# RolandFaure/Hairsplitter

Hardware: AMD Instinct MI355X
Metric: aligned read-bp/sec through call_variants+separate_reads (higher is better)
Workload: dtype u8

## Files before the change

hairsplitter_amd/api.py:

```python
from __future__ import annotations

import ctypes as C
import os
from typing import Dict, List, Optional, Sequence

import numpy as np

from .dist import mean_of_positive_f32, stage4_error_rate, window_size_counts, window_size_from_counts

_ROOT = os.path.dirname(os.path.abspath(__file__))
LIB_PATH = os.path.join(_ROOT, "lib", "libhairsplitter_hip.so")
if os.environ.get("HS_LIB_AB"):
    LIB_PATH = os.environ["HS_LIB_AB"]

SYMBOLS = [
    "hs_cv_batch_set_ploidy", "hs_version", "hs_last_error", "hs_device_count", "hs_warmup", "hs_set_device", "hs_device_synchronize", "hs_malloc", "hs_free",
    "hs_memcpy_h2d", "hs_memcpy_d2h", "hs_memset", "hs_event_create", "hs_event_destroy", "hs_event_record",
    "hs_event_elapsed_ms", "hs_pileup", "hs_pileup_plan", "hs_free_host", "hs_tile_plan", "hs_column_stats_tiled", "hs_cv_column_pass_taps", "hs_cv_taps_destroy", "hs_cv_pileup_tap", "hs_cv_pileup_tap_destroy", "hs_sr_run_taps", "hs_sr_taps_destroy", "hs_exclusive_scan_i32", "hs_gaf_from_files", "hs_gaf_from_labels", "hs_gro_to_gaf_main", "hs_column_partition_test", "hs_column_partition_last_counts", "hs_loop_a_test", "hs_loop_a_result_destroy", "hs_partition_pair_distance", "hs_snp_planes", "hs_simdiff", "hs_read_graphs",
    "hs_edit_distance", "hs_cv_batch_create", "hs_cv_batch_destroy", "hs_cv_batch_aligned_bp", "hs_cv_run",
    "hs_cv_result_destroy", "hs_cv_select", "hs_cv_run_range", "hs_cv_selection_destroy", "hs_sr_run", "hs_sr_run_cv", "hs_sr_run_cv_range", "hs_pipeline_create", "hs_pipeline_select", "hs_pipeline_run", "hs_pipeline_destroy", "hs_pipeline_thread_devices", "hs_cv_batch_device", "hs_sr_result_destroy", "hs_sr_window_size", "hs_call_variants_main", "hs_call_variants_epilogue",
    "hs_pipeline_run_fused", "hs_realign_paf", "hs_pipeline_set_option", "hs_pipeline_groups", "hs_pipeline_group_range", "hs_pipeline_group_cv", "hs_pipeline_sparse_labels", "hs_separate_reads_main", "hs_main_process_exits", "hs_kernel_name", "hs_kernel_stats_reset", "hs_kernel_stats_get", "hs_kernel_stats_every", "hs_host_wait_stats", "hs_devices", "hs_cv_run_host", "hs_edlib_hw_align", "hs_edlib_align", "hs_edlib_align_bytes", "hs_alignment_to_cigar", "hs_reattach_ends", "hs_trim_polished", "hs_reattach_ends_bytes", "hs_trim_polished_bytes", "hs_free_strings", "hs_cut_gfa", "hs_gfa_to_fasta", "hs_cut_gfa_main", "hs_gfa2fa_main",
    "hs_polish_inputs", "hs_polish_inputs_from_files", "hs_polish_result_destroy", "hs_polish_inputs_main",
    "hs_moves_to_cigar", "hs_realign_intervals", "hs_realign_records_destroy", "hs_cv_batch_create_paf", "hs_cv_batch_create_sam",
    "hs_allele_table_destroy", "hs_alleles_text", "hs_alleles_lds_capacity", "hs_group_alleles_layout", "hs_group_alleles", "hs_haplotype_alleles", "hs_pipeline_alleles",
# ... 516 lines not shown
    _fields_ = [("n_snps", C.c_int64), ("n_cw_instances", C.c_int64), ("n_graph_rows_host", C.c_int64),
                ("t_device_ms", C.c_double), ("t_host_ms", C.c_double), ("t_kernel_cv_ms", C.c_float * 4), ("t_kernel_k4_ms", C.c_float),
                ("t_kernel_sr_ms", C.c_float * 4), ("t_kernel_graph_ms", C.c_float),
                ("n_columns_extracted", C.c_int64), ("n_columns_downloaded", C.c_int64), ("n_columns_downloaded_late", C.c_int64),
                ("n_cw_sweeps", C.c_int64), ("cw_bytes", C.c_int64), ("graph_nnz", C.c_int64), ("n_graph_rows", C.c_int64), ("simdiff_bytes", C.c_int64)]


class PipelineGroups:

    def __init__(self, contigs, n_groups):
        self.flat = contigs if isinstance(contigs, FlatBatch) else FlatBatch(contigs)
        self.batch = CvBatch(self.flat)
        self.handle = C.c_void_p()
        _check(load().hs_pipeline_create(self.batch.handle, C.c_int32(n_groups), C.byref(self.handle)))
        self.aligned_bp = self.flat.aligned_bp
        self.total_len = int(self.flat.contig_off[-1])
        self._owns_batch = True

    def keep_columns(self, on=True):
        _check(load().hs_pipeline_set_option(self.handle, C.c_int32(1), C.c_int64(1 if on else 0)))

    def sparse_labels(self, on=True):
        _check(load().hs_pipeline_set_option(self.handle, C.c_int32(2), C.c_int64(1 if on else 0)))
        self._sparse = bool(on)

    def alleles(self, on=True):
        _check(load().hs_pipeline_set_option(self.handle, C.c_int32(4), C.c_int64(1 if on else 0)))
        self._alleles = bool(on)

    def recruits(self, on=True, params=None):
        if params is not None:
            _check(load().hs_pipeline_set_recruit_params(self.handle, C.byref(_recruit_params(params))))
        _check(load().hs_pipeline_set_option(self.handle, C.c_int32(8), C.c_int64(1 if on else 0)))
        self._recruits = bool(on)

    def _attach_sparse(self, sr):
        if getattr(self, "_recruits", False):
            tb = load().hs_pipeline_recruits(self.handle)
            if not tb:
                raise HsError("hs_pipeline_recruits: no table")
            sr["recruits"] = _recruit_table_to_dict(tb)
        if getattr(self, "_alleles", False):
            tb = load().hs_pipeline_alleles(self.handle)
            if not tb:
                raise HsError("hs_pipeline_alleles: no table")
            sr["alleles"] = _allele_table_to_dict(tb)
        if not getattr(self, "_sparse", False):
            return sr
        off, ids, lab = C.POINTER(C.c_int64)(), C.POINTER(C.c_int32)(), C.POINTER(C.c_int32)()
        nw, nr = C.c_int64(0), C.c_int64(0)
        _check(load().hs_pipeline_sparse_labels(self.handle, C.byref(off), C.byref(ids), C.byref(lab), C.byref(nw), C.byref(nr)))
        W, R = int(nw.value), int(nr.value)
        if R == 0:
            sr["sparse"] = (np.ctypeslib.as_array(off, (W + 1,)), np.zeros(0, np.int32), np.zeros(0, np.int32))
            return sr
        sr["sparse"] = (np.ctypeslib.as_array(off, (W + 1,)), np.ctypeslib.as_array(ids, (R,)), np.ctypeslib.as_array(lab, (R,)))
        return sr

    def sibling(self, n_groups):
        o = object.__new__(PipelineGroups)
        o.flat, o.batch, o.aligned_bp, o.total_len = self.flat, self.batch, self.aligned_bp, self.total_len
        o.handle = C.c_void_p()
        o._owns_batch = False
        _check(load().hs_pipeline_create(self.batch.handle, C.c_int32(n_groups), C.byref(o.handle)))
        return o

    def run(self, automatic_snp_threshold=0.33, n_threads=0, error_rate_fn=None, rarest_strain_abundance=0.01, low_memory=False,
            amplicon=False, seed=12345, window_size=0):
        import time
        lib = load()
        Cn = self.flat.n_contigs
        md = np.zeros(max(Cn, 1), np.float32)
        st = PipelineStats()
        t_0 = time.perf_counter()
        _check(lib.hs_pipeline_select(self.handle, _hp(md, C.c_float), C.byref(st)))
        t_1 = time.perf_counter()
        md = md[:Cn]
        cv = {"mean_distance": md, "error_rate": mean_of_positive_f32(md)}
        e = error_rate_fn(cv) if error_rate_fn is not None else stage4_error_rate(cv["error_rate"])
        sres = C.POINTER(SrResult)()
        t_2 = time.perf_counter()
        _check(lib.hs_pipeline_run(self.handle, C.c_float(automatic_snp_threshold), C.c_float(e), C.c_float(rarest_strain_abundance),
                                   C.c_int32(1 if low_memory else 0), C.c_int32(1 if amplicon else 0), C.c_uint32(seed), C.c_int32(n_threads),
                                   C.c_int32(window_size), C.byref(sres), C.byref(st)))
        t_3 = time.perf_counter()
        cv.update({"n_snps": int(st.n_snps), "t_device_ms": float(st.t_device_ms), "t_host_ms": float(st.t_host_ms),
                   "t_kernel_ms": [float(x) for x in st.t_kernel_cv_ms], "t_kernel_k4_ms": float(st.t_kernel_k4_ms),
                   "n_columns_extracted": int(st.n_columns_extracted), "n_columns_downloaded": int(st.n_columns_downloaded),
                   "n_columns_downloaded_late": int(st.n_columns_downloaded_late)})
        sr = self._attach_sparse(_sr_result_to_dict(sres, Cn, take_ownership=True))
        sr["wall_ms"] = {"select": (t_1 - t_0) * 1e3, "between": (t_2 - t_1) * 1e3, "groups": (t_3 - t_2) * 1e3, "collect": (time.perf_counter() - t_3) * 1e3}
        return cv, sr

    def run_fused(self, automatic_snp_threshold=0.33, n_threads=0, rarest_strain_abundance=0.01, low_memory=False, amplicon=False, seed=12345,
                  window_size=0):
        import time
        lib = load()
        Cn = self.flat.n_contigs
        md = np.zeros(max(Cn, 1), np.float32)
        st = PipelineStats()
        er = C.c_float(0)
        sres = C.POINTER(SrResult)()
        t_0 = time.perf_counter()
        _check(lib.hs_pipeline_run_fused(self.handle, C.c_float(automatic_snp_threshold), C.c_float(rarest_strain_abundance), C.c_int32(1 if low_memory else 0),
                                         C.c_int32(1 if amplicon else 0), C.c_uint32(seed), C.c_int32(n_threads), C.c_int32(window_size), _hp(md, C.c_float),
                                         C.byref(er), C.byref(sres), C.byref(st)))
        t_1 = time.perf_counter()
        cv = {"mean_distance": md[:Cn], "error_rate": float(er.value), "error_rate_is_final": True, "n_snps": int(st.n_snps), "t_device_ms": float(st.t_device_ms),
              "t_host_ms": float(st.t_host_ms), "t_kernel_ms": [float(x) for x in st.t_kernel_cv_ms], "t_kernel_k4_ms": float(st.t_kernel_k4_ms),
              "n_columns_extracted": int(st.n_columns_extracted), "n_columns_downloaded": int(st.n_columns_downloaded),
              "n_columns_downloaded_late": int(st.n_columns_downloaded_late)}
        sr = self._attach_sparse(_sr_result_to_dict(sres, Cn, take_ownership=True))
        sr["wall_ms"] = {"select": 0.0, "between": 0.0, "groups": (t_1 - t_0) * 1e3, "collect": (time.perf_counter() - t_1) * 1e3}
        return cv, sr

    def window_size(self, amplicon=False):
        f = self.flat
        if amplicon:
            return int(np.diff(f.contig_off).max()) if f.n_contigs else 0
        return window_size_from_counts(*window_size_counts(f.rec_refspan + 2))

    def close(self):
        if self.handle:
            load().hs_pipeline_destroy(self.handle)
            self.handle = None
        if getattr(self, "_owns_batch", True):
            self.batch.close()


class _SrResultOwner:

    def __init__(self, res):
        self.res = res

    def __del__(self):
        try:
            load().hs_sr_result_destroy(self.res)
        except Exception:
            pass


class _SrTaps(C.Structure):
    _fields_ = [("n_windows", C.c_int32), ("win_contig", C.POINTER(C.c_int32)), ("win_start", C.POINTER(C.c_int32)), ("win_row0", C.POINTER(C.c_int64)),
                ("mask_ids", C.POINTER(C.c_int32)), ("run_begin", C.POINTER(C.c_int64)), ("run_snp", C.POINTER(C.c_int32)), ("run_off", C.POINTER(C.c_int64)),
                ("run_labels", C.POINTER(C.c_int32)), ("third", C.POINTER(C.c_int32)),
                ("g_n_windows", C.c_int32), ("g_win_contig", C.POINTER(C.c_int32)), ("g_win_kind", C.POINTER(C.c_int32)), ("g_win_row0", C.POINTER(C.c_int64)),
                ("g_mask_ids", C.POINTER(C.c_int32)), ("g_nbr_off", C.POINTER(C.c_int64)), ("g_nbr", C.POINTER(C.c_int32)), ("g_n_contigs", C.c_int32),
                ("g_plane_n", C.POINTER(C.c_int32)), ("g_words", C.POINTER(C.c_int32)), ("g_plane_off", C.POINTER(C.c_int64)), ("g_alt", C.POINTER(C.c_uint64)),
                ("g_ref", C.POINTER(C.c_uint64)), ("g_n_reads", C.POINTER(C.c_int32)), ("g_out_off", C.POINTER(C.c_int64)), ("g_read_base", C.POINTER(C.c_int64)),
                ("g_pos_orig", C.POINTER(C.c_int32)), ("g_n_pos_orig", C.c_int64), ("g_n_plane_words", C.c_int64), ("g_n_pairs", C.c_int64),
                ("g_matrix", C.POINTER(C.c_int32)), ("g_rows_on_host", C.c_int64), ("g_rows_late", C.c_int64), ("g_row_waves", C.c_int32),
                ("all_lanes", C.c_int32), ("cap_tail", C.c_int32), ("runs_lanes", C.c_int64), ("runs_overflow", C.c_int64), ("runs_rows", C.c_int64),
                ("units_rows", C.c_int64), ("runs_wave", C.c_int64), ("runs_wave_scratch", C.c_int64), ("tail_narrow", C.c_int64), ("tail_lds", C.c_int64),
                ("tail_scratch", C.c_int64)]


SR_ROUTE_COUNTERS = ("all_lanes", "runs_lanes", "runs_overflow", "runs_rows", "units_rows", "runs_wave", "runs_wave_scratch", "tail_narrow", "tail_lds",
                     "tail_scratch", "cap_tail")


SR_TAP_SENTINEL = -2 ** 31


def _sr_run_taps_fn(lib):
    lib.hs_sr_run_taps.argtypes = [C.c_void_p, C.c_int32, C.c_int32, C.c_float, C.c_int32, C.c_uint32, C.c_int32, C.c_int32, C.POINTER(C.POINTER(SrResult)),
                                   C.POINTER(C.POINTER(_SrTaps))]
    lib.hs_sr_taps_destroy.argtypes = [C.POINTER(_SrTaps)]; lib.hs_sr_taps_destroy.restype = None
    return lib.hs_sr_run_taps


def _graph_taps_to_dict(t):
    a = lambda ptr, n, dt: np.ctypeslib.as_array(ptr, (max(n, 1),))[:n].astype(dt).copy()
    W, Cn = int(t.g_n_windows), int(t.g_n_contigs)
    row0 = a(t.g_win_row0, W + 1, np.int64)
    rows = int(row0[-1])
    noff = a(t.g_nbr_off, rows + 1, np.int64)
    return {"win_contig": a(t.g_win_contig, W, np.int32), "win_kind": a(t.g_win_kind, W, np.int32), "win_row0": row0, "mask_ids": a(t.g_mask_ids, rows, np.int32),
            "nbr_off": noff, "nbr": a(t.g_nbr, int(noff[-1]), np.int32),
            "plane_n": a(t.g_plane_n, Cn, np.int32), "words": a(t.g_words, Cn, np.int32), "plane_off": a(t.g_plane_off, Cn, np.int64),
            "alt": a(t.g_alt, int(t.g_n_plane_words), np.uint64), "ref": a(t.g_ref, int(t.g_n_plane_words), np.uint64),
            "n_reads": a(t.g_n_reads, Cn, np.int32), "out_off": a(t.g_out_off, Cn, np.int64), "read_base": a(t.g_read_base, Cn, np.int64),
            "pos_orig": a(t.g_pos_orig, int(t.g_n_pos_orig), np.int32), "matrix": a(t.g_matrix, 2 * int(t.g_n_pairs), np.int32).reshape(-1, 2),
            "rows_on_host": int(t.g_rows_on_host), "rows_late": int(t.g_rows_late), "row_waves": int(t.g_row_waves)}


def _sr_contig_array(contigs):
    Cn = len(contigs)
    arr = (SrContig * max(Cn, 1))()
    keep = []
    for c, ctg in enumerate(contigs):
        rs, re = _np(ctg["read_start"], np.int32), _np(ctg["read_end"], np.int32)
        sp, sr, sa = _np(ctg["snp_pos"], np.int32), _np(ctg["snp_ref"], np.uint8), _np(ctg["snp_alt"], np.uint8)
        co, ci, cc = _np(ctg["col_off"], np.int64), _np(ctg["col_idx"], np.int32), _np(ctg["col_code"], np.uint8)
        if len(ci) == 0:
            ci, cc = np.zeros(1, np.int32), np.zeros(1, np.uint8)
        keep += [rs, re, sp, sr, sa, co, ci, cc]
        a = arr[c]
        a.length = int(ctg["length"]); a.n_reads = len(rs); a.n_snps = len(sp)
        a.read_start = _hp(rs, C.c_int32); a.read_end = _hp(re, C.c_int32)
        a.snp_pos = _hp(sp, C.c_int32); a.snp_ref = _hp(sr, C.c_uint8); a.snp_alt = _hp(sa, C.c_uint8)
        a.col_off = _hp(co, C.c_int64); a.col_idx = _hp(ci, C.c_int32); a.col_code = _hp(cc, C.c_uint8)
        a.ploidy = 0
    return arr, keep


def separate_reads_graph_taps(contigs: Sequence[Dict], window_size: int, error_rate: float, low_memory: bool = False, seed: int = 12345,
                              n_threads: int = 0) -> Dict:
    require_gpu()
    lib = load()
    Cn = len(contigs)
    arr, keep = _sr_contig_array(contigs)
    res = C.POINTER(SrResult)()
    tp = C.POINTER(_SrTaps)()
    _check(_sr_run_taps_fn(lib)(C.cast(arr, C.c_void_p), C.c_int32(Cn), C.c_int32(int(window_size)), C.c_float(error_rate), C.c_int32(1 if low_memory else 0),
                                C.c_uint32(seed), C.c_int32(n_threads), C.c_int32(1), C.byref(res), C.byref(tp)))
    out = _graph_taps_to_dict(tp.contents)
    lib.hs_sr_taps_destroy(tp)
    return out


def _chain_taps_to_dict(t):
    a = lambda ptr, n, dt: np.ctypeslib.as_array(ptr, (max(n, 1),))[:n].astype(dt).copy()
    Wc = int(t.n_windows)
    row0 = a(t.win_row0, Wc + 1, np.int64); rb = a(t.run_begin, Wc + 1, np.int64)
    n_runs = int(rb[-1]); ro = a(t.run_off, n_runs + 1, np.int64)
    out = {"win_contig": a(t.win_contig, Wc, np.int32), "win_start": a(t.win_start, Wc, np.int32), "win_row0": row0, "mask_ids": a(t.mask_ids, int(row0[-1]), np.int32),
           "run_begin": rb, "run_snp": a(t.run_snp, n_runs, np.int32), "run_off": ro, "run_labels": a(t.run_labels, int(ro[-1]), np.int32),
           "third": a(t.third, int(row0[-1]), np.int32)}
    for k in SR_ROUTE_COUNTERS:
        out[k] = int(getattr(t, k))
    return out


def separate_reads_chain_taps(contigs: Sequence[Dict], window_size: int, error_rate: float, low_memory: bool = False, seed: int = 12345,
                              n_threads: int = 0) -> Dict:
    require_gpu()
    lib = load()
    Cn = len(contigs)
    arr, keep = _sr_contig_array(contigs)
    res = C.POINTER(SrResult)()
    tp = C.POINTER(_SrTaps)()
    _check(_sr_run_taps_fn(lib)(C.cast(arr, C.c_void_p), C.c_int32(Cn), C.c_int32(int(window_size)), C.c_float(error_rate), C.c_int32(1 if low_memory else 0),
                                C.c_uint32(seed), C.c_int32(n_threads), C.c_int32(0), C.byref(res), C.byref(tp)))
    out = _sr_result_to_dict(res, Cn)
    out["window_size"] = int(window_size)
    lib.hs_sr_result_destroy(res)
    out["taps"] = _chain_taps_to_dict(tp.contents)
    lib.hs_sr_taps_destroy(tp)
    return out


def _sr_result_to_dict(res, Cn, take_ownership=False):
    r = res.contents
    win_off = np.ctypeslib.as_array(r.win_off, (Cn + 1,)).copy()
    W = int(win_off[-1])
    label_off = np.ctypeslib.as_array(r.label_off, (W + 1,)).copy()
    NL = int(label_off[-1])
    return {
        "win_off": win_off,
        "win_start": np.ctypeslib.as_array(r.win_start, (max(W, 1),))[:W].copy(),
        "win_end": np.ctypeslib.as_array(r.win_end, (max(W, 1),))[:W].copy(),
        "label_off": label_off,
        "labels": (None if not r.labels else (_owned_view_i32(res, r.labels, NL) if take_ownership else np.ctypeslib.as_array(r.labels, (max(NL, 1),))[:NL].copy())),
        "_owner": (_SrResultOwner(res) if (take_ownership and not r.labels) else None),
        "t_device_ms": float(r.t_device_ms), "t_host_ms": float(r.t_host_ms), "n_cw_instances": int(r.n_cw_instances),
        "t_kernel_ms": [float(x) for x in r.t_kernel_ms], "t_kernel_graph_ms": float(r.t_kernel_graph_ms),
        "n_graph_rows_host": int(r.n_graph_rows_host), "n_windows_finished_on_host": int(r.n_windows_finished_on_host),
        "n_cw_sweeps": int(r.n_cw_sweeps), "cw_bytes": int(r.cw_bytes), "graph_nnz": int(r.graph_nnz), "n_graph_rows": int(r.n_graph_rows),
        "simdiff_bytes": int(r.simdiff_bytes),
    }


def _owned_view_i32(res, ptr, n):
    buf = (C.c_int32 * max(n, 1)).from_address(C.addressof(ptr.contents))
    buf._hs_owner = _SrResultOwner(res)
    return np.ctypeslib.as_array(buf)[:n]


def separate_reads(cv_out: Dict, flat: FlatBatch, error_rate: float, low_memory: bool = False, amplicon: bool = False,
                   seed: int = 12345, n_threads: int = 0, ploidy: Optional[Sequence[int]] = None,
                   rarest_strain_abundance: float = 0.0, window_size: Optional[int] = None, taps: bool = False, alleles: bool = False,
                   recruit=False) -> Dict:
    require_gpu()
    lib = load()
    Cn = flat.n_contigs
    arr = (SrContig * Cn)()
    keep = []
    per_contig = []
    ops = flat.cigar & 0xF
    lens = (flat.cigar >> 4).astype(np.int64)
    refc = np.where((ops == 0) | (ops == 2) | (ops == 7) | (ops == 8), lens, 0)
    csum = np.concatenate(([0], np.cumsum(refc)))
    span = csum[flat.rec_cig_off[1:]] - csum[flat.rec_cig_off[:-1]]
    for c in range(Cn):
        r0, r1 = int(flat.contig_rec_off[c]), int(flat.contig_rec_off[c + 1])
        rs = _np(flat.rec_pos[r0:r1], np.int32)
        re = _np(flat.rec_pos[r0:r1].astype(np.int64) + 1 + span[r0:r1], np.int32)
        s0, s1 = int(cv_out["snp_off"][c]), int(cv_out["snp_off"][c + 1])
        e0 = int(cv_out["col_off"][s0])
        snp_pos = _np(cv_out["snp_pos"][s0:s1], np.int32)
        snp_ref = _np(cv_out["snp_ref"][s0:s1], np.uint8)
        snp_alt = _np(cv_out["snp_alt"][s0:s1], np.uint8)
        col_off = _np(cv_out["col_off"][s0:s1 + 1] - e0, np.int64)
        e1 = e0 + int(col_off[-1])
        col_idx = _np(cv_out["col_idx"][e0:e1], np.int32)
        col_code = _np(cv_out["col_code"][e0:e1], np.uint8)
        if rarest_strain_abundance > 0 and s1 > s0:
            seg = np.repeat(np.arange(s1 - s0), np.diff(col_off))
            n_ref = np.bincount(seg, weights=(col_code == snp_ref[seg]), minlength=s1 - s0)
            n_alt = np.bincount(seg, weights=(col_code == snp_alt[seg]) & (col_code != snp_ref[seg]), minlength=s1 - s0)
            keep_snp = n_alt.astype(np.float32) >= np.float32(rarest_strain_abundance) * (n_ref + n_alt).astype(np.float32)
            if not keep_snp.all():
                km = keep_snp[seg]
                lens = np.diff(col_off)[keep_snp]
                snp_pos, snp_ref, snp_alt = snp_pos[keep_snp], snp_ref[keep_snp], snp_alt[keep_snp]
                col_idx, col_code = _np(col_idx[km], np.int32), _np(col_code[km], np.uint8)
                col_off = _np(np.concatenate(([0], np.cumsum(lens))), np.int64)
                snp_pos, snp_ref, snp_alt = _np(snp_pos, np.int32), _np(snp_ref, np.uint8), _np(snp_alt, np.uint8)
                s1 = s0 + len(snp_pos)
        keep += [rs, re, snp_pos, snp_ref, snp_alt, col_off, col_idx, col_code]
        per_contig.append({"read_start": rs, "read_end": re, "snp_pos": snp_pos, "snp_ref": snp_ref, "snp_alt": snp_alt, "col_off": col_off, "col_idx": col_idx,
                           "col_code": col_code, "length": int(flat.contig_off[c + 1] - flat.contig_off[c])})
        a = arr[c]
        a.length = int(flat.contig_off[c + 1] - flat.contig_off[c])
        a.n_reads = r1 - r0
        a.read_start = _hp(rs, C.c_int32); a.read_end = _hp(re, C.c_int32)
        a.n_snps = s1 - s0
        a.snp_pos = _hp(snp_pos, C.c_int32); a.snp_ref = _hp(snp_ref, C.c_uint8); a.snp_alt = _hp(snp_alt, C.c_uint8)
        a.col_off = _hp(col_off, C.c_int64); a.col_idx = _hp(col_idx, C.c_int32); a.col_code = _hp(col_code, C.c_uint8)
        a.ploidy = int(ploidy[c]) if ploidy is not None else 0
    w = lib.hs_sr_window_size(arr, C.c_int32(Cn), C.c_int32(1 if amplicon else 0)) if window_size is None else int(window_size)
    if taps == "graphs":
        return {"window_size": int(w), "contigs": per_contig, "taps": separate_reads_graph_taps(per_contig, int(w), error_rate, low_memory, seed, n_threads)}
    res = C.POINTER(SrResult)()
    tp = C.POINTER(_SrTaps)()
    if taps:
        _check(_sr_run_taps_fn(lib)(C.cast(arr, C.c_void_p), C.c_int32(Cn), C.c_int32(w), C.c_float(error_rate), C.c_int32(1 if low_memory else 0),
                                    C.c_uint32(seed), C.c_int32(n_threads), C.c_int32(0), C.byref(res), C.byref(tp)))
    else:
        _check(lib.hs_sr_run(arr, C.c_int32(Cn), C.c_int32(w), C.c_float(error_rate), C.c_int32(1 if low_memory else 0),
                             C.c_uint32(seed), C.c_int32(n_threads), C.byref(res)))
    r = res.contents
    win_off = np.ctypeslib.as_array(r.win_off, (Cn + 1,)).copy()
    W = int(win_off[-1])
    label_off = np.ctypeslib.as_array(r.label_off, (W + 1,)).copy()
    NL = int(label_off[-1])
    out = {
        "window_size": int(w), "win_off": win_off,
        "win_start": np.ctypeslib.as_array(r.win_start, (max(W, 1),))[:W].copy(),
        "win_end": np.ctypeslib.as_array(r.win_end, (max(W, 1),))[:W].copy(),
        "label_off": label_off,
        "labels": np.ctypeslib.as_array(r.labels, (max(NL, 1),))[:NL].copy(),
        "t_device_ms": float(r.t_device_ms), "t_host_ms": float(r.t_host_ms), "n_cw_instances": int(r.n_cw_instances),
        "t_kernel_ms": [float(x) for x in r.t_kernel_ms], "t_kernel_graph_ms": float(r.t_kernel_graph_ms),
        "n_graph_rows_host": int(r.n_graph_rows_host), "n_windows_finished_on_host": int(r.n_windows_finished_on_host),
        "n_cw_sweeps": int(r.n_cw_sweeps), "cw_bytes": int(r.cw_bytes), "graph_nnz": int(r.graph_nnz), "n_graph_rows": int(r.n_graph_rows),
        "simdiff_bytes": int(r.simdiff_bytes),
    }
    if alleles:
        tb = C.POINTER(AlleleTable)()
        _check(lib.hs_haplotype_alleles(arr, C.c_int32(Cn), res, C.byref(tb)))
        out["alleles"] = _allele_table_to_dict(tb)
        lib.hs_allele_table_destroy(tb)
    if recruit:
        rt = C.POINTER(RecruitTable)()
        prm = _recruit_params(recruit if isinstance(recruit, dict) else None)
        _check(lib.hs_recruit_reads(arr, C.c_int32(Cn), res, C.byref(prm), None, C.byref(rt)))
        out["recruits"] = _recruit_table_to_dict(rt)
        lib.hs_recruit_table_destroy(rt)
    lib.hs_sr_result_destroy(res)
    if taps:
        out["taps"] = _chain_taps_to_dict(tp.contents)
        out["contigs"] = per_contig
        lib.hs_sr_taps_destroy(tp)
    return out


def alleles_lds_capacity() -> int:
    return int(load().hs_alleles_lds_capacity())


def _table_array(ptr, n, dtype) -> np.ndarray:
# ... 1169 lines not shown
```

hairsplitter_amd/csrc/hs_capi_multi.inc:

```
static std::vector<int> device_list() {
    std::vector<int> d;
    if (const char* e = std::getenv("HS_DEVICES")) {
        for (const char* p = e; *p;) { char* end = nullptr; const long v = std::strtol(p, &end, 10); if (end == p) break; d.push_back((int)v); p = *end == ',' ? end + 1 : end; }
    }
    int n = 0;
    if (hipGetDeviceCount(&n) != hipSuccess) n = 0;
    if (d.empty()) for (int i = 0; i < n; ++i) d.push_back(i);
    for (int& v : d) if (v < 0 || v >= n) v = 0;
    return d;
}
int hs_devices(int32_t* out, int32_t cap) {
    const std::vector<int> d = device_list();
    for (size_t i = 0; i < d.size() && (int32_t)i < cap; ++i) out[i] = d[i];
    return (int)d.size();
}
static std::vector<std::vector<int>> lpt_shards(const std::vector<double>& w, int parts) {
    std::vector<int> order(w.size());
    for (size_t i = 0; i < w.size(); ++i) order[i] = (int)i;
    std::sort(order.begin(), order.end(), [&](int a, int b) { return w[(size_t)a] != w[(size_t)b] ? w[(size_t)a] > w[(size_t)b] : a < b; });
    std::vector<double> load((size_t)parts, 0.0);
    std::vector<std::vector<int>> sh((size_t)parts);
    for (int i : order) {
        int best = 0;
        for (int k = 1; k < parts; ++k) if (load[(size_t)k] < load[(size_t)best]) best = k;
        sh[(size_t)best].push_back(i); load[(size_t)best] += w[(size_t)i];
    }
    for (auto& v : sh) std::sort(v.begin(), v.end());
    return sh;
}
static int run_on_devices(const std::vector<int>& devs, const std::function<int(int)>& f) {
    const int D = (int)devs.size();
    std::vector<int> rcs((size_t)D, 0);
    std::vector<std::string> errs((size_t)D);
    std::vector<std::thread> th;
    for (int k = 0; k < D; ++k)
        th.emplace_back([&, k] {
            if (hipSetDevice(devs[(size_t)k]) != hipSuccess) { rcs[(size_t)k] = HS_EHIP; errs[(size_t)k] = "hipSetDevice failed"; return; }
            set_wait_policy();
            rcs[(size_t)k] = f(k);
            if (rcs[(size_t)k]) errs[(size_t)k] = hs_last_error();
        });
    for (auto& t : th) t.join();
    for (int k = 0; k < D; ++k) if (rcs[(size_t)k]) { set_error(errs[(size_t)k]); return rcs[(size_t)k]; }
    return HS_OK;
}

void hs_sr_taps_destroy(hs_sr_taps* t) {
    if (!t) return;
    std::free(t->win_contig); std::free(t->win_start); std::free(t->win_row0); std::free(t->mask_ids); std::free(t->run_begin); std::free(t->run_snp); std::free(t->run_off);
    std::free(t->run_labels); std::free(t->third);
    std::free(t->g_win_contig); std::free(t->g_win_kind); std::free(t->g_win_row0); std::free(t->g_mask_ids); std::free(t->g_nbr_off); std::free(t->g_nbr);
    std::free(t->g_plane_n); std::free(t->g_words); std::free(t->g_plane_off); std::free(t->g_alt); std::free(t->g_ref); std::free(t->g_n_reads); std::free(t->g_out_off);
    std::free(t->g_read_base); std::free(t->g_pos_orig); std::free(t->g_matrix);
    std::free(t);
}
int hs_sr_run_taps(const hs_sr_contig* contigs, int32_t n_contigs, int32_t window_size, float error_rate, int32_t low_memory, uint32_t seed,
                   int32_t n_threads, int32_t mode, hs_sr_result** out, hs_sr_taps** taps) {
    if (int rc = require_device()) return rc;
    if (!out || !taps || n_contigs < 0 || (mode != HS_SR_TAPS_CHAIN && mode != HS_SR_TAPS_GRAPHS)) { set_error("hs_sr_run_taps: bad arguments"); return HS_EINVAL; }
    hs::SrTaps tp;
    tp.graphs = mode == HS_SR_TAPS_GRAPHS;
    {
        HipSrOps ops;
        if (int rc = hs::sr_run(ops, contigs, n_contigs, window_size, error_rate, low_memory, seed, n_threads, out, nullptr, nullptr, &tp)) return rc;
    }
    const size_t Wc = tp.win_contig.size();
    for (size_t k = 0; k < Wc; ++k) {
        const int64_t r0 = tp.win_row0[k], m = tp.win_row0[k + 1] - r0;
        for (int64_t i = tp.run_begin[k]; i < tp.run_begin[k + 1]; ++i)
            for (int64_t j = 0; j < m; ++j) { int32_t& l = tp.run_labels[(size_t)(tp.run_off[(size_t)i] + j)]; if (l >= 0 && l < m) l = tp.mask_ids[(size_t)(r0 + l)]; }
    }
    auto dup_vec = [](const auto& v) { using T = typename std::decay<decltype(v)>::type::value_type; T* p = (T*)std::malloc(std::max<size_t>(1, v.size()) * sizeof(T)); if (p && !v.empty()) std::memcpy(p, v.data(), v.size() * sizeof(T)); return p; };
    hs_sr_taps* t = (hs_sr_taps*)std::calloc(1, sizeof(hs_sr_taps));
    t->n_windows = (int32_t)Wc;
    t->win_contig = dup_vec(tp.win_contig); t->win_start = dup_vec(tp.win_start); t->win_row0 = dup_vec(tp.win_row0); t->mask_ids = dup_vec(tp.mask_ids);
    t->run_begin = dup_vec(tp.run_begin); t->run_snp = dup_vec(tp.run_snp); t->run_off = dup_vec(tp.run_off); t->run_labels = dup_vec(tp.run_labels); t->third = dup_vec(tp.third);
    {
        const hs::SrChainRoutes& rt = tp.routes;
        t->all_lanes = rt.all_lanes; t->cap_tail = rt.cap_tail; t->runs_lanes = rt.runs_lanes; t->runs_overflow = rt.runs_overflow; t->runs_rows = rt.runs_rows;
        t->units_rows = rt.units_rows; t->runs_wave = rt.runs_wave; t->runs_wave_scratch = rt.runs_wave_scratch; t->tail_narrow = rt.tail_narrow;
        t->tail_lds = rt.tail_lds; t->tail_scratch = rt.tail_scratch;
    }
    if (tp.graphs) {
        const hs::SrGraphTaps& f = tp.front;
        t->g_n_windows = (int32_t)f.win_contig.size();
        t->g_win_contig = dup_vec(f.win_contig); t->g_win_kind = dup_vec(f.win_kind); t->g_win_row0 = dup_vec(f.win_row0); t->g_mask_ids = dup_vec(f.mask_ids);
        t->g_nbr_off = dup_vec(f.nbr_off); t->g_nbr = dup_vec(f.nbr);
        t->g_n_contigs = (int32_t)f.plane_n.size();
        t->g_plane_n = dup_vec(f.plane_n); t->g_words = dup_vec(f.words); t->g_plane_off = dup_vec(f.plane_off); t->g_alt = dup_vec(f.alt); t->g_ref = dup_vec(f.ref);
        t->g_n_reads = dup_vec(f.n_reads); t->g_out_off = dup_vec(f.out_off); t->g_read_base = dup_vec(f.read_base); t->g_pos_orig = dup_vec(f.pos_orig);
        t->g_n_pos_orig = (int64_t)f.pos_orig.size(); t->g_n_plane_words = (int64_t)f.alt.size(); t->g_n_pairs = (int64_t)f.matrix.size() / 2;
        t->g_matrix = dup_vec(f.matrix);
        t->g_rows_on_host = f.rows_on_host; t->g_rows_late = f.rows_late; t->g_row_waves = f.row_waves;
    }
    *taps = t;
    return HS_OK;
}

int hs_sr_run(const hs_sr_contig* contigs, int32_t n_contigs, int32_t window_size, float error_rate, int32_t low_memory,
              uint32_t seed, int32_t n_threads, hs_sr_result** out) {
    if (int rc = require_device()) return rc;
    if (!out || n_contigs < 0) { set_error("hs_sr_run: bad arguments"); return HS_EINVAL; }
    const std::vector<int> devs = device_list();
    if (devs.size() <= 1 || n_contigs < 2) {
        HipSrOps ops;
        return hs::sr_run(ops, contigs, n_contigs, window_size, error_rate, low_memory, seed, n_threads, out);
    }
    std::vector<double> w((size_t)n_contigs);
    for (int c = 0; c < n_contigs; ++c) w[(size_t)c] = 16.0 * contigs[c].n_reads * (double)contigs[c].n_reads + (double)contigs[c].n_snps * contigs[c].n_reads + 1.0;
    const int D = (int)std::min<size_t>(devs.size(), (size_t)n_contigs);
    const std::vector<std::vector<int>> shards = lpt_shards(w, D);
    std::vector<hs_sr_result*> parts((size_t)D, nullptr);
    const int per = n_threads > 0 ? std::max(1, n_threads / D) : 0;
    const int rc = run_on_devices(std::vector<int>(devs.begin(), devs.begin() + D), [&](int k) {
        std::vector<hs_sr_contig> sub;
        for (int c : shards[(size_t)k]) sub.push_back(contigs[c]);
        HipSrOps ops;
        return hs::sr_run(ops, sub.data(), (int32_t)sub.size(), window_size, error_rate, low_memory, seed, per, &parts[(size_t)k]);
    });
    if (rc) { for (hs_sr_result* r : parts) if (r) hs::free_sr_result(r); return rc; }
    std::vector<std::pair<int, int>> where((size_t)n_contigs);
    for (int k = 0; k < D; ++k) for (size_t i = 0; i < shards[(size_t)k].size(); ++i) where[(size_t)shards[(size_t)k][i]] = std::make_pair(k, (int)i);
    hs_sr_result* R = (hs_sr_result*)std::calloc(1, sizeof(hs_sr_result));
    int64_t W = 0, NL = 0;
    for (hs_sr_result* r : parts) { W += r->win_off[r->n_contigs]; NL += r->label_off[r->win_off[r->n_contigs]]; }
    R->n_contigs = n_contigs;
    R->win_off = (int64_t*)std::malloc(((size_t)n_contigs + 1) * sizeof(int64_t));
    R->win_start = (int32_t*)std::malloc((size_t)std::max<int64_t>(1, W) * sizeof(int32_t));
    R->win_end = (int32_t*)std::malloc((size_t)std::max<int64_t>(1, W) * sizeof(int32_t));
    R->label_off = (int64_t*)std::malloc(((size_t)W + 1) * sizeof(int64_t));
    R->labels = hs::sr_labels_alloc((size_t)NL);
    R->win_off[0] = 0; R->label_off[0] = 0;
    std::vector<int64_t> lab0((size_t)n_contigs + 1, 0);
    for (int c = 0; c < n_contigs; ++c) {
        const hs_sr_result* r = parts[(size_t)where[(size_t)c].first];
        const int i = where[(size_t)c].second;
        R->win_off[c + 1] = R->win_off[c] + (r->win_off[i + 1] - r->win_off[i]);
        lab0[(size_t)c + 1] = lab0[(size_t)c] + (r->label_off[r->win_off[i + 1]] - r->label_off[r->win_off[i]]);
    }
    R->label_off[W] = NL;
    hs::hs_parallel_for(n_contigs, host_threads(), [&](int c) {
        const hs_sr_result* r = parts[(size_t)where[(size_t)c].first];
        const int i = where[(size_t)c].second;
        const int64_t q0 = r->win_off[i], nq = r->win_off[i + 1] - q0, w0 = R->win_off[c];
        if (nq == 0) return;
        std::memcpy(R->win_start + w0, r->win_start + q0, (size_t)nq * sizeof(int32_t));
        std::memcpy(R->win_end + w0, r->win_end + q0, (size_t)nq * sizeof(int32_t));
        const int64_t shift = lab0[(size_t)c] - r->label_off[q0];
        for (int64_t q = 0; q < nq; ++q) R->label_off[w0 + q] = r->label_off[q0 + q] + shift;
        std::memcpy(R->labels + lab0[(size_t)c], r->labels + r->label_off[q0], (size_t)(r->label_off[q0 + nq] - r->label_off[q0]) * sizeof(int32_t));
    });
    for (hs_sr_result* r : parts) {
        R->t_device_ms += r->t_device_ms; R->t_host_ms += r->t_host_ms; R->n_cw_instances += r->n_cw_instances;
        for (int k = 0; k < 4; ++k) R->t_kernel_ms[k] += r->t_kernel_ms[k];
        R->t_kernel_graph_ms += r->t_kernel_graph_ms; R->n_graph_rows_host += r->n_graph_rows_host; R->n_windows_finished_on_host += r->n_windows_finished_on_host;
        R->n_cw_sweeps += r->n_cw_sweeps; R->cw_bytes += r->cw_bytes; R->graph_nnz += r->graph_nnz; R->n_graph_rows += r->n_graph_rows; R->simdiff_bytes += r->simdiff_bytes;
        hs::free_sr_result(r);
    }
    *out = R;
    return HS_OK;
}

int hs_cv_run_host(const uint8_t* h_contig_seq, const int64_t* h_contig_off, int32_t n_contigs, const uint8_t* h_read_seq, const int64_t* h_read_off,
                   int32_t n_reads, const int32_t* h_rec_read, const int32_t* h_rec_pos, const uint8_t* h_rec_strand, const int64_t* h_rec_cig_off,
                   const uint32_t* h_cigar, const int32_t* h_contig_rec_off, float automatic_snp_threshold, int32_t n_threads, hs_cv_result** out) {
    if (int rc = require_device()) return rc;
    if (!out || n_contigs < 0) { set_error("hs_cv_run_host: bad arguments"); return HS_EINVAL; }
    const std::vector<int> devs = device_list();
    if (devs.size() <= 1 || n_contigs < 2) {
        hs_cv_batch* b = nullptr;
        if (int rc = hs_cv_batch_create(h_contig_seq, h_contig_off, n_contigs, h_read_seq, h_read_off, n_reads, h_rec_read, h_rec_pos, h_rec_strand,
                                        h_rec_cig_off, h_cigar, h_contig_rec_off, &b)) return rc;
        const int rc = hs_cv_run(b, automatic_snp_threshold, n_threads, out);
        hs_cv_batch_destroy(b);
        return rc;
    }
    std::vector<double> w((size_t)n_contigs, 1.0);
    for (int c = 0; c < n_contigs; ++c)
        for (int r = h_contig_rec_off[c]; r < h_contig_rec_off[c + 1]; ++r) w[(size_t)c] += (double)(h_read_off[h_rec_read[r] + 1] - h_read_off[h_rec_read[r]]);
    const int D = (int)std::min<size_t>(devs.size(), (size_t)n_contigs);
    const std::vector<std::vector<int>> shards = lpt_shards(w, D);
    std::vector<hs_cv_result*> parts((size_t)D, nullptr);
    const int per = n_threads > 0 ? std::max(1, n_threads / D) : 0;
    const int rc = run_on_devices(std::vector<int>(devs.begin(), devs.begin() + D), [&](int k) {
        const std::vector<int>& ids = shards[(size_t)k];
        std::vector<int64_t> c_off(1, 0), r_off(1, 0), cig_off(1, 0);
        std::vector<int32_t> rec_off(1, 0), rec_read, rec_pos;
        std::vector<uint8_t> rec_strand;
        std::vector<uint8_t, hs::NoInitAlloc<uint8_t>> c_seq, r_seq;
        std::vector<uint32_t, hs::NoInitAlloc<uint32_t>> cig;
        std::vector<int32_t> new_id((size_t)n_reads, -1);
        int n_sub_reads = 0;
        int64_t c_total = 0, r_total = 0, cig_total = 0, rec_total = 0;
        for (int c : ids) {
            c_total += h_contig_off[c + 1] - h_contig_off[c];
            for (int r = h_contig_rec_off[c]; r < h_contig_rec_off[c + 1]; ++r) {
                rec_total++; cig_total += h_rec_cig_off[r + 1] - h_rec_cig_off[r];
                if (new_id[(size_t)h_rec_read[r]] < 0) { new_id[(size_t)h_rec_read[r]] = n_sub_reads++; r_total += h_read_off[h_rec_read[r] + 1] - h_read_off[h_rec_read[r]]; }
            }
        }
        c_seq.resize((size_t)c_total); r_seq.resize((size_t)r_total); cig.resize((size_t)cig_total);
        rec_read.reserve((size_t)rec_total); rec_pos.reserve((size_t)rec_total); rec_strand.reserve((size_t)rec_total);
        r_off.assign((size_t)n_sub_reads + 1, 0);
        std::fill(new_id.begin(), new_id.end(), -1);
        n_sub_reads = 0;
        int64_t cw = 0, rw = 0, gw = 0;
        for (int c : ids) {
            const int64_t L = h_contig_off[c + 1] - h_contig_off[c];
            std::memcpy(c_seq.data() + cw, h_contig_seq + h_contig_off[c], (size_t)L); cw += L; c_off.push_back(cw);
            for (int r = h_contig_rec_off[c]; r < h_contig_rec_off[c + 1]; ++r) {
                const int g = h_rec_read[r];
                if (new_id[(size_t)g] < 0) {
                    new_id[(size_t)g] = n_sub_reads;
                    const int64_t n = h_read_off[g + 1] - h_read_off[g];
                    std::memcpy(r_seq.data() + rw, h_read_seq + h_read_off[g], (size_t)n); rw += n;
                    r_off[(size_t)++n_sub_reads] = rw;
                }
                rec_read.push_back(new_id[(size_t)g]); rec_pos.push_back(h_rec_pos[r]); rec_strand.push_back(h_rec_strand[r]);
                const int64_t n = h_rec_cig_off[r + 1] - h_rec_cig_off[r];
                std::memcpy(cig.data() + gw, h_cigar + h_rec_cig_off[r], (size_t)n * sizeof(uint32_t)); gw += n; cig_off.push_back(gw);
            }
            rec_off.push_back((int32_t)rec_read.size());
        }
        hs_cv_batch* b = nullptr;
        if (int rc2 = hs_cv_batch_create(c_seq.data(), c_off.data(), (int32_t)ids.size(), r_seq.data(), r_off.data(), n_sub_reads, rec_read.data(), rec_pos.data(),
                                         rec_strand.data(), cig_off.data(), cig.data(), rec_off.data(), &b)) return rc2;
        const int rc2 = hs_cv_run(b, automatic_snp_threshold, per, &parts[(size_t)k]);
        hs_cv_batch_destroy(b);
        return rc2;
    });
    if (rc) { for (hs_cv_result* r : parts) if (r) hs::free_cv_result(r); return rc; }
    std::vector<std::pair<int, int>> where((size_t)n_contigs);
    for (int k = 0; k < D; ++k) for (size_t i = 0; i < shards[(size_t)k].size(); ++i) where[(size_t)shards[(size_t)k][i]] = std::make_pair(k, (int)i);
    hs_cv_result* R = (hs_cv_result*)std::calloc(1, sizeof(hs_cv_result));
// ... 55 lines not shown
```

hairsplitter_amd/csrc/hs_driver.h:

```cpp
#pragma once
#include <cstdint>
#include <functional>
#include <vector>
#include "hs_host.h"
#include "hs_host_sr.h"

namespace hs {

struct CvMeta {
    int32_t n_contigs = 0, n_rec = 0;
    std::vector<int64_t> contig_off;
    std::vector<int32_t> contig_rec_off;
    std::vector<int64_t> pile_off;
    std::vector<int32_t> rec_pos;
    std::vector<int64_t> rec_refspan;
    int64_t total_len = 0;
    std::vector<int32_t> ploidy;
    std::vector<int32_t> rank_of, orig_of;
};

struct CvPartitionTest {
    std::vector<int32_t> contig_n_reads;
    std::vector<int32_t> part_off;
    std::vector<int64_t> part_state_off;
    std::vector<int8_t> part_state;
};

struct CvCandidates {
    int64_t n_columns = 0, n_entries = 0;
    int64_t n_tie = 0, n_tie_big = 0;
    std::vector<int32_t> contig_n_cand;
    std::vector<float> contig_mean_distance;
    int64_t n_cand = 0;
    const hs_colrec* rec = nullptr;
    const int32_t* col = nullptr;
    const int64_t* off = nullptr;
    const int32_t* idx = nullptr;
    const uint8_t* code = nullptr;
    const CandBits* bits = nullptr;
    const uint64_t* words = nullptr;
    std::vector<uint8_t> contig_on_device;
};
struct CvSnpSet {
    std::vector<int32_t> contig_n_snp;
    int64_t n_snp = 0, n_entries = 0;
    const hs_colrec* rec = nullptr;
    const int64_t* off = nullptr;
    const int32_t* idx = nullptr;
    const uint8_t* code = nullptr;
};

struct CvLoopAResult {
    std::vector<uint8_t> on_device;
    std::vector<int32_t> failed;
    std::vector<int64_t> part_base;
    const CvPartRecord* rec = nullptr;
    const uint64_t* bits = nullptr;
    const int32_t* cnt = nullptr;
};

struct CvDeviceOps {
    virtual ~CvDeviceOps() {}
    virtual int pileup(std::vector<int32_t>& rec_stats, float k_ms[4]) = 0;
    virtual int extract_candidates(int c0, int c1, const std::vector<int32_t>& min_reads, float automatic_snp_threshold, CvCandidates& out,
                                   float k_ms[3], bool want_entries = true) = 0;
    virtual int fetch_candidates(CvCandidates& out) { (void)out; return -1; }
    virtual int finish_columns(const CvPartitionTest& t, bool want_entries, CvSnpSet& out, float* k_ms) = 0;
    virtual int late_entries(CvSnpSet& out) { (void)out; return 0; }
    virtual bool has_partition_pairs() const { return false; }
    virtual int partition_pairs(const std::vector<int8_t>& state, const std::vector<int32_t>& more, const std::vector<int32_t>& less, const std::vector<int64_t>& part_off,
                                const std::vector<int32_t>& part_n, const std::vector<int32_t>& pair_a, const std::vector<int32_t>& pair_b, const std::vector<float>& sigma3,
                                std::vector<int32_t>& out) { (void)state; (void)more; (void)less; (void)part_off; (void)part_n; (void)pair_a; (void)pair_b; (void)sigma3; (void)out; return -1; }
    virtual int collect_partitions(CvLoopAResult& out) { out = CvLoopAResult(); return 0; }
};

struct CvSelection {
    std::vector<int32_t> rec_stats;
    float k_ms[4] = {0, 0, 0, 0};
    double t_device_ms = 0, t_host_ms = 0;
};
int cv_pileup(CvDeviceOps& dev, const CvMeta& meta, CvSelection& sel);
int cv_run_range(CvDeviceOps& dev, const CvMeta& meta, const std::vector<int32_t>& rec_stats, int c0, int c1, float automatic_snp_threshold, int n_threads,
                 hs_cv_result** out, bool resident = false, const std::function<void(const float*)>* on_mean_distance = nullptr);
int cv_run(CvDeviceOps& dev, const CvMeta& meta, float automatic_snp_threshold, int n_threads, hs_cv_result** out);
hs_cv_result* cv_concat_results(hs_cv_result* a, hs_cv_result* b);
int cv_attach_entries(CvDeviceOps& dev, hs_cv_result* r, int n_threads, bool borrow = false);

struct SrWindowSet {
    std::vector<int32_t> win_contig;
    std::vector<int64_t> win_row0;
    std::vector<int32_t> mask_ids;
    int32_t n_dev_windows = 0;
    int32_t n_matrix_windows = 0;
    std::vector<int32_t> ctg_reads;
    std::vector<int64_t> host_off;
    std::vector<int32_t> host_nbr;
    std::vector<uint8_t> win_final_empty;
    std::vector<int32_t> rank;
    std::vector<int32_t> pos_rank;
    std::vector<int64_t> ctg_rank_off;
    float error_rate = 0;
    int64_t rows() const { return win_row0.empty() ? 0 : win_row0.back(); }
};

template <class T> struct ArrayView {
    const T* p = nullptr;
    size_t n = 0;
    std::vector<T> own;
    void view(const T* ptr, size_t count) { own.clear(); p = ptr; n = count; }
    T* alloc(size_t count) { own.resize(count); p = own.data(); n = count; return own.data(); }
    const T* data() const { return p; }
    size_t size() const { return n; }
    const T& operator[](size_t i) const { return p[i]; }
};

struct CwChain {
    ArrayView<int64_t> col_off;
    ArrayView<int32_t> col_idx;
    ArrayView<uint8_t> col_code;
    std::vector<int32_t> win;
    std::vector<int64_t> chain_row0;
    std::vector<int64_t> win_seed_begin;
    std::vector<int64_t> seed_col;
    bool finish_on_device = false;
    std::vector<int32_t> col_pos;
    std::vector<int64_t> win_snp_first, win_snp_last;
    std::vector<int32_t> win_pos_lo, win_pos_hi;
};

struct CwWave {
    std::vector<int32_t> inst_win;
    std::vector<int64_t> inst_label_off;
    std::vector<int32_t> labels;
};

struct SimdiffJob {
    const CwChain* cols = nullptr;
    std::vector<uint8_t> snp_ref, snp_alt;
    std::vector<int32_t> snp_contig;
    std::vector<int64_t> contig_snp_base;
    std::vector<int64_t> plane_off, out_off;
    std::vector<int32_t> n_reads, words;
    std::vector<int32_t> plane_n;
    int64_t plane_total = 0, out_total = 0;
    std::vector<int32_t> pos_orig;
    std::vector<int64_t> read_base;
};

struct SrChainStats {
    int64_t n_instances = 0;
    int64_t sweeps = 0;
    int64_t bytes = 0;
    int64_t graph_nnz = 0;
};

struct SrGraphTaps;
struct SrChainRoutes {
    int32_t all_lanes = 0;
    int64_t runs_lanes = 0;
    int64_t runs_overflow = 0;
    int64_t runs_rows = 0;
    int64_t units_rows = 0;
    int64_t runs_wave = 0;
    int64_t runs_wave_scratch = 0;
    int64_t tail_narrow = 0;
    int64_t tail_lds = 0;
    int64_t tail_scratch = 0;
    int32_t cap_tail = 0;
};
struct SrDeviceOps {
    virtual ~SrDeviceOps() {}
    virtual int simdiff_columns(const SimdiffJob& job, float* k_ms) = 0;
    virtual int build_graphs(const SrWindowSet& ws, int64_t* rows_on_host, float* k_ms) = 0;
    virtual bool two_phase_graphs() const { return false; }
    virtual int build_graphs_begin(const SrWindowSet& ws, float* k_ms) { (void)ws; (void)k_ms; return -1; }
    virtual int build_graphs_end(const SrWindowSet& ws, int64_t* rows_on_host) { (void)ws; (void)rows_on_host; return -1; }
    virtual int fetch_graphs(std::vector<int64_t>& off, std::vector<int32_t>& nbr) = 0;
    virtual int cw_chain(const CwChain& chain, std::vector<int32_t>& labels, std::vector<int32_t>& final_labels,
                         std::vector<uint8_t>& final_ok, float k_ms[3], SrChainStats* stats) = 0;
    virtual int cw(CwWave& wave, float* k_ms) = 0;
    virtual void tap_chain(std::vector<int64_t>* run_off, std::vector<int32_t>* run_labels, SrChainRoutes* routes) { (void)run_off; (void)run_labels; (void)routes; }
    virtual void tap_front(SrGraphTaps* t) { (void)t; }
    virtual bool low_memory_graphs() const { return false; }
    virtual bool columns_resident() const { return false; }
    virtual void drop_resident_columns() {}
    virtual int window_masks(const std::vector<int64_t>& col_a, const std::vector<int64_t>& col_b, const std::vector<int64_t>& slot_off,
                             std::vector<int32_t>& ids, std::vector<int32_t>& win_m) { (void)col_a; (void)col_b; (void)slot_off; (void)ids; (void)win_m; return -1; }
    virtual int fetch_columns(std::vector<int32_t>& idx, std::vector<uint8_t>& code) { (void)idx; (void)code; return -1; }
};

void set_trace_origin();
double trace_ms();
int host_threads();

struct SrSparseLabels {
    std::vector<int64_t> off;
    std::vector<int32_t> ids, labels;
};
struct SrWorkspace { std::vector<SrContigState> st; };
struct SrGraphTaps {
    static constexpr int32_t kSentinel = INT32_MIN;
    std::vector<int32_t> win_contig, win_kind;
    std::vector<int64_t> win_row0;
    std::vector<int32_t> mask_ids;
    std::vector<int64_t> nbr_off;
    std::vector<int32_t> nbr;
    std::vector<int32_t> plane_n, words, n_reads;
    std::vector<int64_t> plane_off, out_off, read_base;
    std::vector<int32_t> pos_orig;
    std::vector<uint64_t> alt, ref;
    std::vector<int32_t> matrix;
    int64_t rows_on_host = 0, rows_late = 0;
    int32_t row_waves = 0;
};
struct SrTaps {
    std::vector<int32_t> win_contig, win_start;
    std::vector<int64_t> win_row0;
    std::vector<int32_t> mask_ids;
    std::vector<int64_t> run_begin;
    std::vector<int32_t> run_snp;
    std::vector<int64_t> run_off;
    std::vector<int32_t> run_labels, third;
    SrChainRoutes routes;
    bool graphs = false;
    SrGraphTaps front;
};
int sr_run(SrDeviceOps& dev, const hs_sr_contig* contigs, int32_t n_contigs, int32_t window_size, float error_rate,
           int32_t low_memory, uint32_t seed, int32_t n_threads, hs_sr_result** out, SrSparseLabels* sparse = nullptr, SrWorkspace* keep = nullptr, SrTaps* taps = nullptr);

inline bool snp_kept_by_abundance(int32_t n_ref, int32_t n_alt, float rarest_strain_abundance) {
    return (float)n_alt >= rarest_strain_abundance * (float)(n_ref + n_alt);
}
int sr_run_from_cv(SrDeviceOps& dev, const CvMeta& meta, int c0, int c1, const hs_cv_result* cv, float error_rate, float rarest_strain_abundance,
                   int32_t low_memory, int32_t amplicon, uint32_t seed, int32_t n_threads, int32_t window_size, hs_sr_result** out,
                   SrSparseLabels* sparse = nullptr, SrWorkspace* keep = nullptr);

int32_t* sr_labels_alloc(size_t n_labels);
void sr_labels_free(int32_t* labels);
void sr_expand_labels(const SrSparseLabels& sp, const int64_t* label_off, int64_t w0, int64_t w1, int32_t* dense);

struct ColFileContig {
    std::string contig_line, name;
    long length = 0;
    std::vector<std::string> read_lines;
    std::vector<int32_t> read_start, read_end;
    std::vector<int32_t> snp_pos;
    std::vector<uint8_t> snp_ref, snp_alt;
    std::vector<int64_t> col_off{0};
    std::vector<int32_t> col_idx;
    std::vector<uint8_t> col_code;
};
int parse_col(const std::string& path, float rarest_strain_abundance, std::vector<ColFileContig>& cs, int n_threads = 1);
int read_col_sidecar(const std::string& col_path, float rarest_strain_abundance, std::vector<ColFileContig>& cs, int n_threads = 1);

int write_cv_outputs(const CvFileInput& in, const hs_cv_result* res, const std::string& error_rate_out,
                     const std::string& col_path, const std::string& vcf_path, int n_threads = 1);
int write_gro(const std::vector<ColFileContig>& cs, const hs_sr_result* res, const std::string& path, int n_threads = 1);
int write_gro_companion(const std::string& col_path, const std::vector<ColFileContig>& cs, const hs_sr_result* res, float error_rate, float rsa, bool low_memory, bool amplicon,
                        uint32_t seed, int32_t window, int n_threads);
int take_gro_companion(const std::string& col_path, float error_rate, float rsa, bool low_memory, bool amplicon, uint32_t seed, const std::string& outfile, int n_threads);
void remove_gro_companion(const std::string& col_path);
bool mark_gro_companion_pending(const std::string& col_path, float error_rate, float rsa, bool low_memory, bool amplicon, uint32_t seed);

void free_cv_result(hs_cv_result* r);
void free_sr_result(hs_sr_result* r);

}
```

hairsplitter_amd/csrc/hs_kernels_cw.hip:

```cpp
#pragma once

namespace hsdev {

#define HS_FIN_KCAP 16
#define HS_FIN_GCAP 8
#define HS_FIN_LCAP 16
#define HS_FIN_MCAP (HS_FIN_KCAP + 2)
#define HS_TAIL_MAP_EXTRA 1024
#define HS_TAIL_BATCH 8
#define HS_CWR_CAP 255
#ifndef HS_CW_REG_LABELS
#define HS_CW_REG_LABELS 8
#endif

static __device__ __forceinline__ int local_index(const int32_t* __restrict__ ids, int m, int r) {
    int lo = 0, hi = m;
    while (lo < hi) { const int mid = (lo + hi) >> 1; if (ids[mid] < r) lo = mid + 1; else hi = mid; }
    return (lo < m && ids[lo] == r) ? lo : -1;
}

__global__ __launch_bounds__(256) void k_cw_visit_lists(
    const int64_t* __restrict__ off, const int32_t* __restrict__ nbr, const int64_t* __restrict__ win_row0, const int32_t* __restrict__ mask_ids,
    const int32_t* __restrict__ win_contig, const int64_t* __restrict__ ctg_rank_off, const int32_t* __restrict__ rank,
    int n_windows, int cap, int32_t* __restrict__ visit, int32_t* __restrict__ visit_n,
// ... 239 lines not shown
                const int nc = __builtin_amdgcn_readfirstlane((int)((inf >> 8) & 255u));
                const uint8_t* pg = s_prog + (inf >> 16) * 16 + l;
                unsigned best = 0u;
                const int old = (int)lab[i];
                if (nc == 1) {
                    const int n0 = pg[0];
                    const int lb = n0 != 255 ? (int)lab[n0] : -1;
                    int cnt = 1;
#define HS_ROT(K) { const int o = __builtin_amdgcn_update_dpp(-2, lb, 0x120 + (K), 0xf, 0xf, false); cnt += o == lb ? 1 : 0; }
                    HS_ROT(1) HS_ROT(2) HS_ROT(3) HS_ROT(4) HS_ROT(5) HS_ROT(6) HS_ROT(7) HS_ROT(8)
                    HS_ROT(9) HS_ROT(10) HS_ROT(11) HS_ROT(12) HS_ROT(13) HS_ROT(14) HS_ROT(15)
#undef HS_ROT
                    best = row_max_u32(lb >= 0 ? (((unsigned)cnt << 16) | (unsigned)(65535 - lb)) : 0u);
                } else if (nc <= 4) {
                    const int n0 = pg[0], n1 = pg[16], n2 = nc > 2 ? pg[32] : 255, n3 = nc > 3 ? pg[48] : 255;
                    int lb0 = n0 != 255 ? (int)lab[n0] : -1, lb1 = n1 != 255 ? (int)lab[n1] : -1;
                    int lb2 = n2 != 255 ? (int)lab[n2 & 255] : -1, lb3 = n3 != 255 ? (int)lab[n3 & 255] : -1;
                    const int sh = tid & 48;
                    bool left = true;
                    for (int round = 0; round < HS_CW_REG_LABELS; ++round) {
                        const int mine = lb0 >= 0 ? lb0 : (lb1 >= 0 ? lb1 : (lb2 >= 0 ? lb2 : lb3));
                        const unsigned key = row_max_u32((unsigned)(mine + 1));
                        if (__ballot(key != 0u) == 0ull) { left = false; break; }
                        const int X = (int)key - 1;
                        const unsigned long long b0 = __ballot(lb0 == X && X >= 0), b1 = __ballot(lb1 == X && X >= 0);
                        const unsigned long long b2 = __ballot(lb2 == X && X >= 0), b3 = __ballot(lb3 == X && X >= 0);
                        const int c = __popc((unsigned)(b0 >> sh) & 0xffffu) + __popc((unsigned)(b1 >> sh) & 0xffffu) + __popc((unsigned)(b2 >> sh) & 0xffffu)
                                    + __popc((unsigned)(b3 >> sh) & 0xffffu);
                        const unsigned k = X >= 0 ? (((unsigned)c << 16) | (unsigned)(65535 - X)) : 0u;
                        best = k > best ? k : best;
                        lb0 = lb0 == X ? -1 : lb0; lb1 = lb1 == X ? -1 : lb1; lb2 = lb2 == X ? -1 : lb2; lb3 = lb3 == X ? -1 : lb3;
                    }
                    if (left && __ballot((lb0 & lb1 & lb2 & lb3) >= 0 || lb0 >= 0 || lb1 >= 0 || lb2 >= 0 || lb3 >= 0) != 0ull) {
                        const int m0 = n0 != 255 ? (int)lab[n0] : -1, m1 = n1 != 255 ? (int)lab[n1] : -1, m2 = n2 != 255 ? (int)lab[n2 & 255] : -1, m3 = n3 != 255 ? (int)lab[n3 & 255] : -1;
                        best = 0u;
                        if (m0 >= 0) atomicAdd(&cnt[m0], 1);
                        if (m1 >= 0) atomicAdd(&cnt[m1], 1);
                        if (m2 >= 0) atomicAdd(&cnt[m2], 1);
                        if (m3 >= 0) atomicAdd(&cnt[m3], 1);
                        wave_lds_sync();
                        if (m0 >= 0) { const unsigned k = ((unsigned)cnt[m0] << 16) | (unsigned)(65535 - m0); best = k > best ? k : best; }
                        if (m1 >= 0) { const unsigned k = ((unsigned)cnt[m1] << 16) | (unsigned)(65535 - m1); best = k > best ? k : best; }
                        if (m2 >= 0) { const unsigned k = ((unsigned)cnt[m2] << 16) | (unsigned)(65535 - m2); best = k > best ? k : best; }
                        if (m3 >= 0) { const unsigned k = ((unsigned)cnt[m3] << 16) | (unsigned)(65535 - m3); best = k > best ? k : best; }
                        best = row_max_u32(best);
                        wave_lds_sync();
                        if (m0 >= 0) cnt[m0] = 0;
                        if (m1 >= 0) cnt[m1] = 0;
                        if (m2 >= 0) cnt[m2] = 0;
                        if (m3 >= 0) cnt[m3] = 0;
                    }
                } else {
                    for (int c = 0; c < nc; ++c) { const int nb = pg[c * 16]; if (nb != 255) atomicAdd(&cnt[lab[nb]], 1); }
                    wave_lds_sync();
                    for (int c = 0; c < nc; ++c) { const int nb = pg[c * 16]; if (nb != 255) { const int lb = lab[nb]; const unsigned k = ((unsigned)cnt[lb] << 16) | (unsigned)(65535 - lb); best = k > best ? k : best; } }
                    best = row_max_u32(best);
                    wave_lds_sync();
                    for (int c = 0; c < nc; ++c) { const int nb = pg[c * 16]; if (nb != 255) cnt[lab[nb]] = 0; }
                }
                const int best_lab = 65535 - (int)(best & 0xffffu);
                changes += old != best_lab ? 1 : 0;
                wave_lds_sync();
                if (l == 0 && active) lab[i] = (uint8_t)best_lab;
                wave_lds_sync();
                inf = inf_next;
            }
            if (active) { iters++; active = changes > 2 && iters < 15; }
        }
    } else {
        int changes = 3;
        while (live && changes > 2 && iters < 15) {
            changes = 0;
            for (int v = 0; v < n_visit; ++v) {
                const int i = vis[v];
                const int o0 = (int)(off_w[i] - base), o1 = (int)(off_w[i + 1] - base);
                unsigned best = 0u;
                for (int o = o0 + l; o < o1; o += 16) atomicAdd(&cnt[lab[anb[o]]], 1);
                wave_lds_sync();
                for (int o = o0 + l; o < o1; o += 16) { const int lb = lab[anb[o]]; const unsigned key = ((unsigned)cnt[lb] << 16) | (unsigned)(65535 - lb); best = key > best ? key : best; }
                best = row_max_u32(best);
                wave_lds_sync();
                for (int o = o0 + l; o < o1; o += 16) cnt[lab[anb[o]]] = 0;
                const int best_lab = 65535 - (int)(best & 0xffffu);
                if ((int)lab[i] != best_lab) changes++;
                wave_lds_sync();
                if (l == 0) lab[i] = (uint8_t)best_lab;
                wave_lds_sync();
            }
            iters++;
        }
    }
    if (live) {
        int32_t* __restrict__ out = slab + inst_slab_off[inst];
        for (int j = l; j < m; j += 16) out[j] = (int32_t)lab[j];
        if (l == 0 && stat) {
            atomicAdd(&stat[0], (unsigned long long)iters);
            atomicAdd(&stat[1], (unsigned long long)iters * (4ull * (unsigned long long)(off_w[m] - base) + 8ull * (unsigned long long)m));
            atomicAdd(&stat[4 + (iters > 15 ? 15 : iters)], 1ull);
        }
    }
}

__global__ __launch_bounds__(64) void k_cw_seeded_wave(
    const int64_t* __restrict__ off, const int32_t* __restrict__ nbr, const int64_t* __restrict__ win_row0,
    const int32_t* __restrict__ mask_ids, const int32_t* __restrict__ visit, const int32_t* __restrict__ visit_n,
    const int32_t* __restrict__ inst_list, int n_list, const int32_t* __restrict__ n_list_dev ,
    const int32_t* __restrict__ inst_win, const int64_t* __restrict__ inst_seed_col,
    const int64_t* __restrict__ inst_slab_off, const int64_t* __restrict__ col_off, const int32_t* __restrict__ col_idx,
    const uint8_t* __restrict__ col_code, int lds_cap, int32_t* __restrict__ gscratch, const int64_t* __restrict__ gscratch_off,
    int32_t* __restrict__ slab, unsigned long long* __restrict__ stat) {
    extern __shared__ int32_t cw_dyn[];
    __shared__ int32_t s_first[256];
    const int lane = lane_id();
    const int n_runs = n_list_dev ? *n_list_dev : n_list;
    for (int k = (int)blockIdx.x; k < n_runs; k += (int)gridDim.x) {
    wave_lds_sync();
    const int inst = inst_list[k];
    const int w = inst_win[inst];
    const int64_t r0 = win_row0[w];
    const int m = (int)(win_row0[w + 1] - r0);
    const int32_t* __restrict__ ids = mask_ids + r0;
    int32_t* lab = m <= lds_cap ? cw_dyn : gscratch + gscratch_off[k];
    int32_t* cnt = lab + (m <= lds_cap ? lds_cap : m);
    for (int j = lane; j < m; j += 64) { lab[j] = j; cnt[j] = 0; }
    for (int j = lane; j < 256; j += 64) s_first[j] = 0x7fffffff;
    wave_lds_sync();
    const int64_t s = inst_seed_col[inst];
    cw_seed_labels<64>(ids, m, col_off[s], col_off[s + 1], col_idx, col_code, s_first, lane);
    wave_lds_sync();
    for (int64_t e = col_off[s] + lane; e < col_off[s + 1]; e += 64) {
        const int j = local_index(ids, m, col_idx[e]);
        if (j >= 0) lab[j] = s_first[col_code[e]];
    }
    wave_lds_sync();
    const int iters = cw_local_wave(off + r0, nbr, visit + r0, visit_n[w], m, lab, cnt, lane);
    int32_t* __restrict__ out = slab + inst_slab_off[inst];
    for (int j = lane; j < m; j += 64) out[j] = lab[j];
    if (lane == 0 && stat) {
        atomicAdd(&stat[0], (unsigned long long)iters);
        atomicAdd(&stat[1], (unsigned long long)iters * (4ull * (unsigned long long)(off[r0 + m] - off[r0]) + 8ull * (unsigned long long)m));
        atomicAdd(&stat[4 + (iters > 15 ? 15 : iters)], 1ull);
    }
    }
}

#define HS_CWL_SLOTS 16

__global__ __launch_bounds__(256) void k_cw_seed_sets(
    const int64_t* __restrict__ win_row0, const int32_t* __restrict__ mask_ids, const int32_t* __restrict__ inst_list, int n_list,
    const int32_t* __restrict__ inst_win, const int64_t* __restrict__ inst_seed_col, const int64_t* __restrict__ col_off,
    const int32_t* __restrict__ col_idx, const uint8_t* __restrict__ col_code,
    unsigned long long* __restrict__ seed_sets , uint8_t* __restrict__ seed_names ,
    uint8_t* __restrict__ seed_slots , uint8_t* __restrict__ seed_n ,
    int32_t* __restrict__ ovf_list, int32_t* __restrict__ ovf_n) {
    __shared__ int32_t s_ids[4][64];
    __shared__ int32_t s_lab[4][64];
    __shared__ int32_t s_first[4][256];
    const int lane = (int)threadIdx.x & 63, wv = (int)threadIdx.x >> 6;
    const int q = (int)blockIdx.x * 4 + wv;
    if (q >= n_list) return;
    int32_t* ids = s_ids[wv]; int32_t* lab = s_lab[wv]; int32_t* first = s_first[wv];
    const int inst = inst_list[q];
    const int w = inst_win[inst];
    const int64_t seed = inst_seed_col[inst];
    const int64_t r0 = win_row0[w];
    const int m = (int)(win_row0[w + 1] - r0);
    const int64_t c0 = col_off[seed], c1 = col_off[seed + 1];
    const int64_t e0 = c0 + lane;
    const int R0 = e0 < c1 ? col_idx[e0] : -1;
    const int code0 = e0 < c1 ? (int)col_code[e0] : 0;
    ids[lane] = lane < m ? mask_ids[r0 + lane] : 0x7fffffff;
    lab[lane] = lane;
    for (int c = lane; c < 256; c += 64) first[c] = 0x7fffffff;
    wave_lds_sync();
    const int j0 = R0 >= 0 ? local_index(ids, m, R0) : -1;
    if (j0 >= 0) atomicMin(&first[code0], j0);
    for (int64_t e = e0 + 64; e < c1; e += 64) { const int j = local_index(ids, m, col_idx[e]); if (j >= 0) atomicMin(&first[col_code[e]], j); }
    wave_lds_sync();
    if (j0 >= 0) lab[j0] = first[code0];
    for (int64_t e = e0 + 64; e < c1; e += 64) { const int j = local_index(ids, m, col_idx[e]); if (j >= 0) lab[j] = first[col_code[e]]; }
    wave_lds_sync();
    const int L = lab[lane];
    const bool node = lane < m;
    const unsigned long long leaders = __ballot(node && L == lane);
    const int alive = __popcll(leaders);
    const int slot = __popcll(leaders & ((1ull << L) - 1ull));
    seed_slots[(int64_t)q * 64 + lane] = (uint8_t)(node ? slot : 0);
    if (alive > HS_CWL_SLOTS) {
        if (lane == 0) { seed_n[q] = 255; ovf_list[atomicAdd(ovf_n, 1)] = inst; }
        return;
    }
    unsigned long long mine = 0ull;
#pragma unroll
    for (int k = 0; k < HS_CWL_SLOTS; ++k) { const unsigned long long S = __ballot(node && slot == k); if (lane == k) mine = S; }
    if (lane < HS_CWL_SLOTS) seed_sets[(int64_t)q * HS_CWL_SLOTS + lane] = mine;
    if (node && L == lane) ids[slot] = lane;
    wave_lds_sync();
    if (lane < HS_CWL_SLOTS) seed_names[(int64_t)q * HS_CWL_SLOTS + lane] = (uint8_t)(lane < alive ? ids[lane] : 0);
    if (lane == 0) seed_n[q] = (uint8_t)alive;
}

template <int NS>
static __device__ __forceinline__ int cwl_sweeps(unsigned (&set_lo)[HS_CWL_SLOTS], unsigned (&set_hi)[HS_CWL_SLOTS], uint8_t* my_slot,
                                                 const unsigned long long* __restrict__ adj_w, const uint32_t* __restrict__ inf_w, int nv, bool ok) {
    int iters = 0;
    bool active = ok;
    while (__ballot(active) != 0ull) {
        int changes = 0;
        unsigned long long adj_n = (active && nv > 0) ? adj_w[0] : 0ull;
        uint32_t inf_n = (active && nv > 0) ? inf_w[0] : 0u;
        for (int v = 0;; ++v) {
            const bool on = active && v < nv;
            if (__ballot(on) == 0ull) break;
            const unsigned long long adj = adj_n;
            const int i = (int)(inf_n & 255u);
            if (active && v + 1 < nv) { adj_n = adj_w[v + 1]; inf_n = inf_w[v + 1]; }
            const int old = (int)my_slot[i];
            const unsigned lo = (unsigned)adj, hi = (unsigned)(adj >> 32);
            unsigned best = 0u;
#pragma unroll
            for (int s = 0; s < NS; ++s) {
                const unsigned c = (unsigned)__popc(lo & set_lo[s]) + (unsigned)__popc(hi & set_hi[s]);
                const unsigned key = (c << 8) | (unsigned)(255 - s);
                best = key > best ? key : best;
            }
            const int b = 255 - (int)(best & 255u);
            const bool chg = on && b != old;
            changes += chg ? 1 : 0;
            if (__ballot(chg) != 0ull) {
                const unsigned long long bit = chg ? 1ull << i : 0ull;
                const unsigned bl = (unsigned)bit, bh = (unsigned)(bit >> 32);
#pragma unroll
                for (int s = 0; s < NS; ++s) {
                    set_lo[s] = (set_lo[s] & ~bl) | (s == b ? bl : 0u);
                    set_hi[s] = (set_hi[s] & ~bh) | (s == b ? bh : 0u);
                }
                if (chg) my_slot[i] = (uint8_t)b;
            }
        }
        if (active) { iters++; active = changes > 2 && iters < 15; }
    }
    return iters;
}

__global__ __launch_bounds__(64) void k_cw_seeded_lanes(
    const int64_t* __restrict__ off, const int64_t* __restrict__ win_row0, const int32_t* __restrict__ visit_n,
    const uint32_t* __restrict__ prog_info, const unsigned long long* __restrict__ prog_adj,
    const int32_t* __restrict__ inst_list, int n_list, const int32_t* __restrict__ inst_win, const int64_t* __restrict__ inst_slab_off,
    const unsigned long long* __restrict__ seed_sets, const uint8_t* __restrict__ seed_names, const uint8_t* __restrict__ seed_slots ,
    const uint8_t* __restrict__ seed_n, int32_t* __restrict__ slab, unsigned long long* __restrict__ stat) {
    __shared__ uint32_t s_slot[64 * 17];
    __shared__ uint32_t s_name[64 * 4];
    __shared__ unsigned int s_hist[16];
    const int lane = (int)threadIdx.x;
    const int q0 = (int)blockIdx.x * 64, q = q0 + lane;
    const bool valid = q < n_list;
    const int inst = valid ? inst_list[q] : 0;
    const int na = valid ? (int)seed_n[q] : 255;
    const bool ok = valid && na != 255;
    const int w = ok ? inst_win[inst] : 0;
    const int64_t r0 = ok ? win_row0[w] : 0;
    const int m = ok ? (int)(win_row0[w + 1] - r0) : 0;
    const int nv = ok ? visit_n[w] : 0;
    const int64_t out0 = ok ? inst_slab_off[inst] : 0;
    unsigned set_lo[HS_CWL_SLOTS], set_hi[HS_CWL_SLOTS];
    {
        const ulonglong2* p = reinterpret_cast<const ulonglong2*>(seed_sets + (int64_t)(valid ? q : 0) * HS_CWL_SLOTS);
#pragma unroll
        for (int k = 0; k < HS_CWL_SLOTS / 2; ++k) {
            const ulonglong2 v = p[k];
            set_lo[2 * k] = ok ? (unsigned)v.x : 0u; set_hi[2 * k] = ok ? (unsigned)(v.x >> 32) : 0u;
            set_lo[2 * k + 1] = ok ? (unsigned)v.y : 0u; set_hi[2 * k + 1] = ok ? (unsigned)(v.y >> 32) : 0u;
        }
        const uint4 nm = reinterpret_cast<const uint4*>(seed_names)[valid ? q : 0];
        s_name[lane * 4 + 0] = nm.x; s_name[lane * 4 + 1] = nm.y; s_name[lane * 4 + 2] = nm.z; s_name[lane * 4 + 3] = nm.w;
        const uint32_t* src = reinterpret_cast<const uint32_t*>(seed_slots + (int64_t)q0 * 64);
#pragma unroll
        for (int k = 0; k < 16; ++k) { const int x = lane + 64 * k; s_slot[(x >> 4) * 17 + (x & 15)] = src[x]; }
        if (lane < 16) s_hist[lane] = 0u;
    }
    wave_lds_sync();
    int nmax = 0;
#pragma unroll
    for (int k = 1; k <= HS_CWL_SLOTS; ++k) if (__ballot(ok && na >= k) != 0ull) nmax = k;
    uint8_t* my_slot = reinterpret_cast<uint8_t*>(s_slot) + lane * 68;
    int iters;
    if (nmax <= 4) iters = cwl_sweeps<4>(set_lo, set_hi, my_slot, prog_adj + r0, prog_info + r0, nv, ok);
    else if (nmax <= 6) iters = cwl_sweeps<6>(set_lo, set_hi, my_slot, prog_adj + r0, prog_info + r0, nv, ok);
    else if (nmax <= 8) iters = cwl_sweeps<8>(set_lo, set_hi, my_slot, prog_adj + r0, prog_info + r0, nv, ok);
    else if (nmax <= 10) iters = cwl_sweeps<10>(set_lo, set_hi, my_slot, prog_adj + r0, prog_info + r0, nv, ok);
    else if (nmax <= 12) iters = cwl_sweeps<12>(set_lo, set_hi, my_slot, prog_adj + r0, prog_info + r0, nv, ok);
    else iters = cwl_sweeps<HS_CWL_SLOTS>(set_lo, set_hi, my_slot, prog_adj + r0, prog_info + r0, nv, ok);
    wave_lds_sync();
    const unsigned long long okm = __ballot(ok);
    const uint8_t* names = reinterpret_cast<const uint8_t*>(s_name);
    const uint8_t* slots = reinterpret_cast<const uint8_t*>(s_slot);
    const int out_lo = (int)(unsigned)out0, out_hi = (int)(out0 >> 32);
    for (int r = 0; r < 64; ++r) {
        if (!((okm >> r) & 1ull)) continue;
        const int m_r = __builtin_amdgcn_readlane(m, r);
        const int64_t o_r = (int64_t)(((unsigned long long)(unsigned)__builtin_amdgcn_readlane(out_hi, r) << 32) | (unsigned)__builtin_amdgcn_readlane(out_lo, r));
        if (lane < m_r) slab[o_r + lane] = (int32_t)names[r * 16 + slots[r * 68 + lane]];
    }
    if (stat) {
        unsigned long long sw = ok ? (unsigned long long)iters : 0ull;
        unsigned long long by = ok ? (unsigned long long)iters * (4ull * (unsigned long long)(off[r0 + m] - off[r0]) + 8ull * (unsigned long long)m) : 0ull;
        if (ok) atomicAdd(&s_hist[iters > 15 ? 15 : iters], 1u);
#pragma unroll
        for (int d = 32; d >= 1; d >>= 1) { sw += __shfl_xor(sw, d, 64); by += __shfl_xor(by, d, 64); }
        wave_lds_sync();
        if (lane == 0) { atomicAdd(&stat[0], sw); atomicAdd(&stat[1], by); }
        if (lane < 16 && s_hist[lane]) atomicAdd(&stat[4 + lane], (unsigned long long)s_hist[lane]);
    }
}

__global__ __launch_bounds__(64) void k_cw_local(
    const int64_t* __restrict__ off, const int32_t* __restrict__ nbr, const int64_t* __restrict__ win_row0,
    const int32_t* __restrict__ visit, const int32_t* __restrict__ visit_n, const uint8_t* __restrict__ win_final_empty,
    const int32_t* __restrict__ inst_win, const int64_t* __restrict__ inst_label_off, int n_inst, int lds_cap,
    int32_t* __restrict__ gscratch, const int64_t* __restrict__ gscratch_off, int32_t* __restrict__ labels_io) {
    extern __shared__ int32_t cw_dyn[];
    const int lane = lane_id();
    const int k = (int)blockIdx.x;
    if (k >= n_inst) return;
    const int w = inst_win[k];
    const int64_t r0 = win_row0[w];
    const int m = (int)(win_row0[w + 1] - r0);
    int32_t* lab = m <= lds_cap ? cw_dyn : gscratch + gscratch_off[k];
    int32_t* cnt = lab + (m <= lds_cap ? lds_cap : m);
    int32_t* __restrict__ io = labels_io + inst_label_off[k];
    for (int j = lane; j < m; j += 64) { lab[j] = io[j]; cnt[j] = 0; }
    wave_lds_sync();
    cw_local_wave(off + r0, nbr, visit + r0, win_final_empty[w] ? 0 : visit_n[w], m, lab, cnt, lane);
    for (int j = lane; j < m; j += 64) io[j] = lab[j];
}

static __device__ __forceinline__ unsigned long long sets_from_labels(int L, unsigned long long* s_sets, int lane) {
    s_sets[lane] = 0ull;
    wave_lds_sync();
    if (L >= 0) atomicOr(&s_sets[L], 1ull << lane);
    wave_lds_sync();
    const unsigned long long S = s_sets[lane];
    wave_lds_sync();
    return S;
}
static __device__ __forceinline__ int sets_renumber(unsigned long long& S, int& L, unsigned long long* s_sets, int* s_relabel, int lane) {
    const int f = S ? __builtin_ctzll(S) : 64;
    const unsigned long long F = wave_or_u64(S ? 1ull << f : 0ull);
    const int nl = S ? __popcll(F & ((1ull << f) - 1ull)) : -1;
    s_sets[lane] = 0ull; s_relabel[lane] = nl;
    wave_lds_sync();
    if (nl >= 0) s_sets[nl] = S;
    const int Ln = L >= 0 ? s_relabel[L] : -1;
    wave_lds_sync();
    S = s_sets[lane]; L = Ln;
    wave_lds_sync();
    return __popcll(F);
}
#define HS_CW_SPEC_LABELS 8
static __device__ int cw_run_sets(unsigned long long adjv, int nodev, unsigned long long adjn, int n_visit, unsigned long long& S, int& L, int lane) {
    int changes = 3, iters = 0;
    while (changes > 2 && iters < 15) {
        changes = 0;
        unsigned long long alive = __ballot(S != 0ull);
        if (__popcll(alive) > HS_CW_SPEC_LABELS) {
            for (int v = 0; v < n_visit; ++v) {
                const unsigned long long adj = readlane_u64(adjv, v);
                const int i = __builtin_amdgcn_readlane(nodev, v);
                const int c = __popcll(adj & S);
                const int best = wave_max_i32(c ? ((c << 6) | (63 - lane)) : 0);
                if (best) {
                    const int bl = 63 - (best & 63);
                    const int old = __builtin_amdgcn_readlane(L, i);
                    if (old != bl) {
                        changes++;
                        const unsigned long long bit = 1ull << i;
                        if (lane == old) S &= ~bit;
                        if (lane == bl) S |= bit;
                        if (lane == i) L = bl;
                    }
                }
            }
        } else {
            int p = 0;
            while (p < n_visit) {
                int best = 0;
                for (unsigned long long am = alive; am; am &= am - 1ull) {
                    const int l = __builtin_ctzll(am);
                    const int c = __popcll(adjn & readlane_u64(S, l));
                    const int key = c ? ((c << 6) | (63 - l)) : 0;
                    best = key > best ? key : best;
                }
                const int wants = 63 - (best & 63);
                const unsigned long long U = __ballot(best != 0 && wants != L);
                const unsigned long long Uv = __ballot(lane >= p && lane < n_visit && ((U >> nodev) & 1ull));
                if (!Uv) break;
                const int v0 = __builtin_ctzll(Uv);
                const int i = __builtin_amdgcn_readlane(nodev, v0);
                const int bl = __builtin_amdgcn_readlane(wants, i), old = __builtin_amdgcn_readlane(L, i);
                const unsigned long long bit = 1ull << i;
                if (lane == old) S &= ~bit;
                if (lane == bl) S |= bit;
                if (lane == i) L = bl;
                changes++;
                p = v0 + 1;
                alive = __ballot(S != 0ull);
            }
        }
        iters++;
    }
    return iters;
}

static __device__ void first_seen_ids_wave(const int32_t* first, int m, int32_t* pre, int32_t* out_id, int lane) {
    int carry = 0;
    for (int b0 = 0; b0 < m; b0 += 64) {
        const int j = b0 + lane;
        const bool f = j < m && first[j] == j;
        const unsigned long long b = __ballot(f);
        if (j < m) pre[j] = carry + __popcll(b & ((1ull << lane) - 1ull));
        carry += __popcll(b);
    }
    wave_lds_sync();
    for (int j = lane; j < m; j += 64) { const int f = first[j]; out_id[j] = f >= 0 ? pre[f] : -1; }
    wave_lds_sync();
}

__global__ __launch_bounds__(64) void k_window_tail(
    const int64_t* __restrict__ off, const int32_t* __restrict__ nbr, const int64_t* __restrict__ win_row0,
    const int32_t* __restrict__ mask_ids, const int32_t* __restrict__ visit, const int32_t* __restrict__ visit_n,
    const uint8_t* __restrict__ win_final_empty, const uint32_t* __restrict__ prog_info, const unsigned long long* __restrict__ prog_adj,
    const int32_t* __restrict__ chain_win, const int64_t* __restrict__ chain_row0, const int64_t* __restrict__ chain_seed_begin,
    const int64_t* __restrict__ chain_slab0, const int32_t* __restrict__ slab, const int32_t* __restrict__ chain_list , int n_chain,
    const int64_t* __restrict__ col_off, const int32_t* __restrict__ col_idx, const uint8_t* __restrict__ col_code,
    const int32_t* __restrict__ col_pos, const int64_t* __restrict__ win_snp_first, const int64_t* __restrict__ win_snp_last,
    const int32_t* __restrict__ win_pos_lo, const int32_t* __restrict__ win_pos_hi, int finish_on_device,
    int lds_cap, int32_t* __restrict__ gscratch, const int64_t* __restrict__ gscratch_off,
    int32_t* __restrict__ labels3_out, int32_t* __restrict__ final_out, uint8_t* __restrict__ ok_out, unsigned long long* __restrict__ stat) {
    extern __shared__ int32_t tail_dyn[];
    __shared__ int s_count[HS_FIN_KCAP], s_initial[HS_FIN_KCAP], s_tested[HS_FIN_KCAP];
    __shared__ int s_index_of[HS_FIN_KCAP], s_slot_of[HS_FIN_KCAP];
    __shared__ int s_glist[HS_FIN_GCAP], s_gidx[HS_FIN_GCAP];
    __shared__ int s_incompat[HS_FIN_GCAP * HS_FIN_GCAP];
    __shared__ int s_link_cnt[HS_FIN_MCAP * HS_FIN_MCAP], s_links_in[HS_FIN_MCAP], s_o2n[HS_FIN_MCAP], s_new_index[HS_FIN_MCAP];
    static_assert(HS_FIN_MCAP * HS_FIN_MCAP >= 256, "the deep-column histogram shares the link matrix's words");
    int* const s_cnts = s_link_cnt;
    __shared__ int s_scalar[8];
    __shared__ unsigned long long s_sets[64];
    __shared__ int s_relabel[64];
    __shared__ int s_lc1[HS_FIN_LCAP], s_lc2[HS_FIN_LCAP];
    __shared__ double s_lr[HS_FIN_LCAP];
    const int lane = lane_id();
    if ((int)blockIdx.x >= n_chain) return;
    const int c = chain_list[blockIdx.x];
    const int w = chain_win[c];
    const int64_t r0 = win_row0[w];
    const int m = (int)(win_row0[w + 1] - r0);
    const int32_t* __restrict__ ids = mask_ids + r0;
    const int64_t* __restrict__ off_w = off + r0;
    const int64_t abase = off_w[0];
    const int32_t* __restrict__ anb = nbr + abase;
    const int32_t* __restrict__ vis = visit + r0;
    const int n_visit = win_final_empty[w] ? 0 : visit_n[w];
    const int K = (int)(chain_seed_begin[c + 1] - chain_seed_begin[c]);
    const int32_t* __restrict__ sl = slab + chain_slab0[c];
    const bool in_lds = m <= lds_cap;
    const int stride = in_lds ? lds_cap : m;
    int32_t* basep = in_lds ? tail_dyn : gscratch + gscratch_off[c];
    double* agg = reinterpret_cast<double*>(basep);
    int32_t* lab = basep + 2 * stride;
    int32_t* nc = lab + stride;
    int32_t* cnt = nc + stride;
    int32_t* t0 = cnt + stride;
    int32_t* t1 = t0 + stride;
    int32_t* __restrict__ l3 = labels3_out + chain_row0[c];
    int32_t* __restrict__ lout = final_out + chain_row0[c];
    auto bail = [&]() { if (lane == 0) ok_out[c] = 0; };
    unsigned long long sweeps = 0;

#ifdef HS_TAIL_DIAG
    unsigned long long tq0 = __builtin_readcyclecounter();
#define HS_TQ(k) { const unsigned long long tq1 = __builtin_readcyclecounter(); if (lane == 0 && stat) atomicAdd(&stat[18 + (k)], tq1 - tq0); tq0 = tq1; }
#else
#define HS_TQ(k)
#endif
    for (int j = lane; j < m; j += 64) t1[j] = ids[j];
    wave_lds_sync();
    for (int j = lane; j < m; j += 64) {
        double a = 0.0, f = 1.0;
        int i = 0;
        for (; i + 16 <= K; i += 16) {
            int lv[16];
#pragma unroll
            for (int u = 0; u < 16; ++u) lv[u] = sl[(int64_t)(i + u) * m + j];
#pragma unroll
            for (int u = 0; u < 16; ++u) { a += (double)t1[lv[u]] * f; f *= 2.0; }
        }
        for (; i + 4 <= K; i += 4) {
            const int l0 = sl[(int64_t)i * m + j], l1 = sl[(int64_t)(i + 1) * m + j], l2 = sl[(int64_t)(i + 2) * m + j], l3v = sl[(int64_t)(i + 3) * m + j];
            a += (double)t1[l0] * f; f *= 2.0; a += (double)t1[l1] * f; f *= 2.0; a += (double)t1[l2] * f; f *= 2.0; a += (double)t1[l3v] * f; f *= 2.0;
        }
        for (; i < K; ++i) { a += (double)t1[sl[(int64_t)i * m + j]] * f; f *= 2.0; }
        agg[j] = a; cnt[j] = 0;
    }
    wave_lds_sync();
    {
        int T = 1;
        while (T <= m) T <<= 1;
        int32_t* tab = nc;
        for (int x = lane; x < T; x += 64) tab[x] = -1;
        wave_lds_sync();
        for (int j = lane; j < m; j += 64) {
            const double a = agg[j];
            const unsigned long long bits = (unsigned long long)__double_as_longlong(a);
            unsigned h = ((unsigned)(bits >> 32) * 0x9E3779B1u ^ (unsigned)bits * 0x85EBCA6Bu);
            h = (h ^ (h >> 15)) & (unsigned)(T - 1);
            for (;;) {
                const int cur = atomicCAS(&tab[h], -1, j);
                if (cur == -1) break;
                if (agg[cur] == a) { atomicMin(&tab[h], j); break; }
                h = (h + 1u) & (unsigned)(T - 1);
            }
            t0[j] = (int)h;
        }
        wave_lds_sync();
        for (int j = lane; j < m; j += 64) t0[j] = tab[t0[j]];
        wave_lds_sync();
        for (int j = lane; j < m; j += 64) cnt[j] = 0;
        wave_lds_sync();
    }
    first_seen_ids_wave(t0, m, t1, lab, lane);
    HS_TQ(0)
    const bool masks = m <= 64 && prog_adj != nullptr;
    wave_lds_sync();
    int Kc = 0;
    unsigned long long fin_S = 0ull, fin_adjn = 0ull;
    int fin_L = -1;
    if (masks) {
        const unsigned long long adjv = lane < n_visit ? prog_adj[r0 + lane] : 0ull;
        const int nodev = lane < n_visit ? (int)(prog_info[r0 + lane] & 255u) : 0;
        int L = lane < m ? lab[lane] : -1;
        s_sets[lane] = 0ull;
        wave_lds_sync();
        if (lane < n_visit) s_sets[nodev] = adjv;
        wave_lds_sync();
        const unsigned long long adjn = s_sets[lane];
        wave_lds_sync();
        unsigned long long S = sets_from_labels(L, s_sets, lane);
        sweeps += (unsigned long long)cw_run_sets(adjv, nodev, adjn, n_visit, S, L, lane);
        {
            const bool small = S != 0ull && __popcll(S) < 5;
            const unsigned long long gone = wave_or_u64(small ? S : 0ull);
            if (small) S = 0ull;
            if ((gone >> lane) & 1ull) L = -1;
            sets_renumber(S, L, s_sets, s_relabel, lane);
        }
        sweeps += (unsigned long long)cw_run_sets(adjv, nodev, adjn, n_visit, S, L, lane);
        if (lane < m) l3[lane] = L;
        if (lane == 0 && stat) {
            atomicAdd(&stat[0], sweeps);
            atomicAdd(&stat[1], sweeps * (4ull * (unsigned long long)(off_w[m] - abase) + 8ull * (unsigned long long)m));
        }
        if (!finish_on_device) { bail(); return; }
        HS_TQ(1)
        Kc = sets_renumber(S, L, s_sets, s_relabel, lane);
        if (Kc > HS_FIN_KCAP) { bail(); return; }
        HS_TQ(2)
        {
            unsigned long long N = S;
            int Lw = L;
            unsigned long long tested = 0ull;
            for (int j = 0; j < m; ++j) {
                const int target = __builtin_amdgcn_readlane(L, j);
                if (target < 0 || ((tested >> target) & 1ull)) continue;
                int changes = 3, iters = 0;
                while (changes > 0 && iters < 10) {
                    changes = 0;
                    int p = 0;
                    while (p < n_visit) {
                        const unsigned long long alive = __ballot(N != 0ull);
                        int best = 0, second = 0;
                        for (unsigned long long am = alive; am; am &= am - 1ull) {
                            const int l = __builtin_ctzll(am);
                            const int c = __popcll(adjn & readlane_u64(N, l));
                            const int key = c > 0 ? ((c << 8) | (255 - l)) : 0;
                            if (key > best) { second = best; best = key; } else if (key > second) second = key;
                        }
                        const int max_value = best >> 8, max_index = best ? 255 - (best & 255) : 0;
                        const int second_value = second >> 8, second_index = second ? 255 - (second & 255) : 0;
                        int to = -1;
                        if (max_value > 0 && max_index != target) to = max_index;
// ... 45 lines not shown
        atomicAdd(&stat[0], sweeps);
        atomicAdd(&stat[1], sweeps * (4ull * (unsigned long long)(off_w[m] - abase) + 8ull * (unsigned long long)m));
    }
    if (!finish_on_device) { bail(); return; }

    HS_TQ(1)
    for (int j = lane; j < m; j += 64) t1[j] = 0x7fffffff;
    wave_lds_sync();
    bool bad_l = false;
    for (int j = lane; j < m; j += 64) { const int l = lab[j]; if (l >= 0) { if (l >= m) bad_l = true; else atomicMin(&t1[l], j); } }
    wave_lds_sync();
    if (__ballot(bad_l) != 0ull) { bail(); return; }
    for (int b0 = 0; b0 < m; b0 += 64) {
        const int j = b0 + lane;
        int f = -1;
        if (j < m) { const int l = lab[j]; f = l >= 0 ? t1[l] : -1; nc[j] = f; }
        Kc += __popcll(__ballot(j < m && f == j));
    }
    wave_lds_sync();
    first_seen_ids_wave(nc, m, t1, lab, lane);
    if (Kc > HS_FIN_KCAP) { bail(); return; }

    HS_TQ(2)
    if (lane < HS_FIN_KCAP) { s_initial[lane] = 0; s_tested[lane] = 0; }
    wave_lds_sync();
    for (int j = lane; j < m; j += 64) { const int l = lab[j]; if (l >= 0) atomicAdd(&s_initial[l], 1); nc[j] = l; }
    wave_lds_sync();
    for (int j = 0; j < m; ++j) {
        const int target = lab[j];
        if (target < 0 || s_tested[target]) continue;
        if (lane < Kc) s_count[lane] = s_initial[lane];
        wave_lds_sync();
        int changes = 3, iters = 0;
        while (changes > 0 && iters < 10) {
            changes = 0;
            for (int k0 = 0; k0 < n_visit; k0 += 64) {
                const int kk = k0 + lane;
                int i_l = 0, o0_l = 0, o1_l = 0;
                if (kk < n_visit) { i_l = vis[kk]; o0_l = (int)(off_w[i_l] - abase); o1_l = (int)(off_w[i_l + 1] - abase); }
                unsigned long long act = __ballot(kk < n_visit && nc[i_l] == target);
                int nb_next = -1;
                if (act) {
                    const int ln = __builtin_ctzll(act);
                    const int q0 = __builtin_amdgcn_readlane(o0_l, ln), q1 = __builtin_amdgcn_readlane(o1_l, ln);
                    if (q0 + lane < q1) nb_next = anb[q0 + lane];
                }
                while (act) {
                    const int l = __builtin_ctzll(act);
                    act &= act - 1ull;
                    const int i = __builtin_amdgcn_readlane(i_l, l);
                    const int o0 = __builtin_amdgcn_readlane(o0_l, l), o1 = __builtin_amdgcn_readlane(o1_l, l);
                    const int nb0 = nb_next;
                    nb_next = -1;
                    if (act) {
                        const int ln = __builtin_ctzll(act);
                        const int q0 = __builtin_amdgcn_readlane(o0_l, ln), q1 = __builtin_amdgcn_readlane(o1_l, ln);
                        if (q0 + lane < q1) nb_next = anb[q0 + lane];
                    }
                    int v = 0;
                    for (int ob = o0; ob < o1; ob += 64) {
                        int lb = -1;
                        if (ob == o0) { if (nb0 >= 0) lb = nc[nb0]; }
                        else if (ob + lane < o1) lb = nc[anb[ob + lane]];
                        unsigned long long rem = __ballot(lb >= 0);
                        while (rem) {
                            const int L = __builtin_amdgcn_readlane(lb, __builtin_ctzll(rem));
                            const unsigned long long msk = __ballot(lb == L);
                            rem &= ~msk;
                            if (lane == L) v += __popcll(msk);
                        }
                    }
                    const int key = v > 0 ? ((v << 8) | (255 - lane)) : 0;
                    const int best = wave_max_i32(key);
                    const int max_value = best >> 8, max_index = best ? 255 - (best & 255) : 0;
                    const int best2 = wave_max_i32((best && lane == max_index) ? 0 : key);
                    const int second_value = best2 >> 8, second_index = best2 ? 255 - (best2 & 255) : 0;
                    if (max_value > 0 && max_index != target) {
                        if (lane == 0) { s_count[target]--; s_count[max_index]++; nc[i] = max_index; }
                        changes++;
                    } else if (max_value > 0 && max_value <= 2 * second_value) {
                        if (lane == 0) { s_count[target]--; s_count[second_index]++; nc[i] = second_index; }
                        changes++;
                    }
                    wave_lds_sync();
                }
            }
            iters++;
        }
        const bool dissolved = s_count[target] == 0;
        wave_lds_sync();
        if (lane == 0) s_tested[target] = 1;
        if (dissolved) {
            for (int q = lane; q < m; q += 64) lab[q] = nc[q];
            if (lane < Kc) s_initial[lane] = s_count[lane];
        } else {
            for (int q = lane; q < m; q += 64) nc[q] = lab[q];
        }
        wave_lds_sync();
    }

    }

    HS_TQ(3)
    if (lane < HS_FIN_KCAP) { s_index_of[lane] = -1; s_slot_of[lane] = -1; }
    wave_lds_sync();
    if (masks) {
        const bool present = fin_S != 0ull;
        const int f = present ? __builtin_ctzll(fin_S) : 0;
        const unsigned long long F = wave_or_u64(present ? 1ull << f : 0ull);
        const unsigned long long pm = __ballot(present);
        const int index = __popcll(F & ((1ull << f) - 1ull)), slot = __popcll(pm & ((1ull << lane) - 1ull));
        if (present && lane < HS_FIN_KCAP) {
            s_index_of[lane] = index;
            if (slot < HS_FIN_GCAP) { s_slot_of[lane] = slot; s_glist[slot] = lane; s_gidx[slot] = index; }
        }
        if (lane == 0) s_scalar[2] = __popcll(pm);
    } else if (lane == 0) {
        int index = 0;
        for (int j = 0; j < m; ++j) { const int cl = lab[j]; if (cl > -1 && s_index_of[cl] < 0) s_index_of[cl] = index++; }
        int G = 0;
        for (int l = 0; l < Kc; ++l) if (s_index_of[l] >= 0) { if (G < HS_FIN_GCAP) { s_slot_of[l] = G; s_glist[G] = l; s_gidx[G] = s_index_of[l]; } G++; }
        s_scalar[2] = G;
    }
    wave_lds_sync();
    const int G = s_scalar[2];
    if (G <= 1) {
        for (int j = lane; j < m; j += 64) lout[j] = 0;
        if (lane == 0) ok_out[c] = 1;
        return;
    }
    if (G > HS_FIN_GCAP) { bail(); return; }
    for (int x = lane; x < G * G; x += 64) s_incompat[x] = 0;
    wave_lds_sync();
    const int pos_lo = win_pos_lo[c], pos_hi = win_pos_hi[c];
    for (int j = lane; j < m; j += 64) t0[j] = ids[j];
    wave_lds_sync();
    const int32_t* ids_l = t0;
    const int id_lo = m > 0 ? ids_l[0] : 0;
    const long long id_range = m > 0 ? (long long)ids_l[m - 1] - id_lo + 1 : 0;
    const long long map_cap = in_lds ? (8ll * stride > HS_TAIL_MAP_EXTRA ? 8ll * stride : (long long)HS_TAIL_MAP_EXTRA) : 0ll;
    const bool use_map = in_lds && id_range <= map_cap;
    uint8_t* smap = 8ll * stride > HS_TAIL_MAP_EXTRA ? reinterpret_cast<uint8_t*>(agg) : reinterpret_cast<uint8_t*>(tail_dyn + 7 * lds_cap);
    if (use_map) {
        for (int x = lane; x < (int)id_range; x += 64) smap[x] = 0xff;
        wave_lds_sync();
        for (int j = lane; j < m; j += 64) { const int cl = lab[j]; if (cl > -1) smap[ids_l[j] - id_lo] = (uint8_t)s_slot_of[cl]; }
        wave_lds_sync();
    }
    HS_TQ(5)
    const int pa = lane < G * G ? lane / G : 0, pb = lane < G * G ? lane % G : 0;
    const bool pair_owner = lane < G * G && s_glist[pa] > s_glist[pb];
    int pair_inc = 0, pair_last = -10;
#ifdef HS_TAIL_DIAG
    unsigned long long dq_fast = 0, dq_slow = 0, dq_keys = 0;
#endif
    auto pairs_update = [&](int p, int major) {
        const bool counts_l = lane < G && major != 0 && major != ' ';
        const unsigned long long cm = __ballot(counts_l);
        bool several = false;
        if (cm) { const int first_max = __builtin_amdgcn_readlane(major, __builtin_ctzll(cm)); several = __ballot(counts_l && major != first_max) != 0ull; }
        if (several) {
            const int ma = __shfl(major, pa, 64), mb = __shfl(major, pb, 64);
            if (pair_owner && ma != ' ' && mb != ' ' && ma != mb && p - pair_last > 10) { pair_inc += 1; pair_last = p; }
        }
    };
    auto snp_fast = [&](int p, int n, int idx, int code) {
        int slot = 0xff;
        if (lane < n) {
            if (use_map) { const long long d = (long long)idx - id_lo; slot = (d >= 0 && d < id_range) ? (int)smap[d] : 0xff; }
            else { const int j = local_index(ids_l, m, idx); const int cl = j >= 0 ? lab[j] : -2; slot = cl > -1 ? s_slot_of[cl] : 0xff; }
        }
        const int key = slot != 0xff ? ((slot << 8) | code) : -1;
        unsigned long long rem = __ballot(key >= 0);
        int t1v = 0, t2v = 0, c1 = -1, nbv = 0;
#ifdef HS_TAIL_DIAG
        dq_fast++;
#endif
        while (rem) {
#ifdef HS_TAIL_DIAG
            dq_keys++;
#endif
            const int k = __builtin_amdgcn_readlane(key, __builtin_ctzll(rem));
            const unsigned long long msk = __ballot(key == k);
            rem &= ~msk;
            const int v = __popcll(msk);
            if (lane == (k >> 8)) { nbv += v; if (v > t1v) { t2v = t1v; t1v = v; c1 = k & 255; } else if (v > t2v) t2v = v; }
        }
        int major = 0;
        if (lane < G && t1v > 0) { major = c1; if (t2v * 2 > t1v || nbv * 0.5 > t1v) major = ' '; }
        pairs_update(p, major);
    };
    auto snp_deep = [&](int p, int64_t e0, int n) {
#ifdef HS_TAIL_DIAG
        dq_slow++;
#endif
        int major = 0;
        for (int i = 0; i < G; ++i) {
#pragma unroll
            for (int q = 0; q < 4; ++q) s_cnts[lane + 64 * q] = 0;
            wave_lds_sync();
            int nb_i = 0;
            for (int64_t eb = e0; eb < e0 + n; eb += 64) {
                const int64_t e = eb + lane;
                bool mine = false;
                if (e < e0 + n) {
                    const int j = local_index(ids_l, m, col_idx[e]);
                    const int cl = j >= 0 ? lab[j] : -2;
                    mine = cl > -1 && s_slot_of[cl] == i;
                    if (mine) atomicAdd(&s_cnts[col_code[e]], 1);
                }
                nb_i += __popcll(__ballot(mine));
            }
            wave_lds_sync();
            int t1v = 0, c1 = -1, t2v = 0;
#pragma unroll
            for (int q = 0; q < 4; ++q) {
                const int cd = lane + 64 * q;
                const int v = s_cnts[cd];
                if (v > t1v) { t2v = t1v; t1v = v; c1 = cd; } else if (v > t2v) t2v = v;
            }
            wave_lds_sync();
            const int top = wave_max_i32((t1v << 8) | (c1 & 255));
            const int mx = top >> 8;
            if (mx == 0) continue;
            const int n_at = __popcll(__ballot(t1v == mx)) + __popcll(__ballot(t2v == mx));
            const int below = wave_max_i32(t1v == mx ? t2v : t1v);
            const int second_max = n_at >= 2 ? mx : below;
            int max_base = top & 255;
            if (second_max * 2 > mx || nb_i * 0.5 > mx) max_base = ' ';
            if (lane == i) major = max_base & 255;
        }
        pairs_update(p, major);
    };
    for (int64_t sb = win_snp_first[c]; sb < win_snp_last[c]; sb += 64) {
        const int64_t s_l = sb + lane;
        const bool s_valid = s_l < win_snp_last[c];
        const int p_l = s_valid ? col_pos[s_l] : 0;
        const int64_t e0_l = s_valid ? col_off[s_l] : 0;
        const int n_l = s_valid ? (int)(col_off[s_l + 1] - e0_l) : 0;
        unsigned long long todo = __ballot(s_valid && p_l >= pos_lo && p_l < pos_hi);
        auto rl_e0 = [&](int l) { return ((int64_t)(unsigned)__builtin_amdgcn_readlane((int)(e0_l >> 32), l) << 32) | (unsigned)__builtin_amdgcn_readlane((int)(e0_l & 0xffffffffll), l); };
        while (todo) {
            int aq[HS_TAIL_BATCH], idx_b[HS_TAIL_BATCH], code_b[HS_TAIL_BATCH];
            bool any_deep = false;
            const unsigned long long batch_todo = todo;
#pragma unroll
            for (int q = 0; q < HS_TAIL_BATCH; ++q) {
                aq[q] = -1; idx_b[q] = -1; code_b[q] = 0;
                if (todo) {
                    aq[q] = __builtin_ctzll(todo);
                    todo &= todo - 1ull;
                    const int64_t e0 = rl_e0(aq[q]);
                    const int n = __builtin_amdgcn_readlane(n_l, aq[q]);
                    any_deep = any_deep || n > 64;
                    if (lane < n) { idx_b[q] = col_idx[e0 + lane]; code_b[q] = col_code[e0 + lane]; }
                }
            }
            if (!any_deep) {
#pragma unroll
                for (int q = 0; q < HS_TAIL_BATCH; ++q) {
                    if (aq[q] < 0) break;
                    snp_fast(__builtin_amdgcn_readlane(p_l, aq[q]), __builtin_amdgcn_readlane(n_l, aq[q]), idx_b[q], code_b[q]);
                }
            } else {
                unsigned long long bt = batch_todo & ~todo;
                while (bt) {
                    const int a = __builtin_ctzll(bt);
                    bt &= bt - 1ull;
                    const int p = __builtin_amdgcn_readlane(p_l, a), n = __builtin_amdgcn_readlane(n_l, a);
                    const int64_t e0 = rl_e0(a);
                    if (n <= 64) { int idx = -1, code = 0; if (lane < n) { idx = col_idx[e0 + lane]; code = col_code[e0 + lane]; } snp_fast(p, n, idx, code); }
                    else snp_deep(p, e0, n);
                }
            }
        }
    }
#ifdef HS_TAIL_DIAG
    if (lane == 0 && stat) { atomicAdd(&stat[18 + 8], dq_fast); atomicAdd(&stat[18 + 9], dq_slow); atomicAdd(&stat[18 + 10], dq_keys); atomicAdd(&stat[18 + 11], use_map ? 1ull : 0ull); atomicAdd(&stat[18 + 12], (unsigned long long)G); }
#endif
    if (pair_owner) { const int i1 = s_gidx[pa], i2 = s_gidx[pb]; s_incompat[i1 * G + i2] = pair_inc; s_incompat[i2 * G + i1] = pair_inc; }
    wave_lds_sync();
    HS_TQ(6)
    const int M = Kc + 2;
    for (int x = lane; x < M * M; x += 64) s_link_cnt[x] = 0;
    if (lane < M) s_links_in[lane] = 0;
    wave_lds_sync();
    if (masks) {
        const int c2 = fin_L + 2;
        const unsigned long long any = wave_or_u64(fin_S);
        const unsigned long long nolabel = ~any & (m >= 64 ? ~0ull : ((1ull << m) - 1ull));
        {
            const int k = __popcll(fin_adjn & nolabel);
            if (k > 0) { if (c2 != 1) atomicAdd(&s_link_cnt[1 * M + c2], k); atomicAdd(&s_links_in[1], k); }
        }
        for (unsigned long long am = __ballot(fin_S != 0ull); am; am &= am - 1ull) {
            const int l = __builtin_ctzll(am);
            const int k = __popcll(fin_adjn & readlane_u64(fin_S, l));
            if (k > 0) { if (l + 2 != c2) atomicAdd(&s_link_cnt[(l + 2) * M + c2], k); atomicAdd(&s_links_in[l + 2], k); }
        }
    } else if (n_visit > 0) {
        for (int q = lane; q < m; q += 64) {
            const int c2 = lab[q] + 2;
            for (int64_t o = off_w[q]; o < off_w[q + 1]; ++o) {
                const int c1 = lab[nbr[o]] + 2;
                if (c1 != c2) atomicAdd(&s_link_cnt[c1 * M + c2], 1);
                atomicAdd(&s_links_in[c1], 1);
            }
        }
    }
    wave_lds_sync();
    HS_TQ(7)
    {
        int nl_all = 0;
        for (int x0 = 0; x0 < M * M; x0 += 64) {
            const int x = x0 + lane;
            const int cv = x < M * M ? s_link_cnt[x] : 0;
            const unsigned long long nz = __ballot(cv > 0);
            const int rank = nl_all + __popcll(nz & ((1ull << lane) - 1ull));
            if (cv > 0 && rank < HS_FIN_LCAP) { const int c1 = x / M, c2 = x % M; s_lc1[rank] = c1 - 2; s_lc2[rank] = c2 - 2; s_lr[rank] = (double)cv / s_links_in[c1]; }
            nl_all += __popcll(nz);
        }
        if (lane == 0) s_scalar[4] = nl_all;
    }
    wave_lds_sync();
    if (lane == 0) {
        int* lc1 = s_lc1; int* lc2 = s_lc2; double* lr = s_lr;
        const int nl = s_scalar[4] > HS_FIN_LCAP ? HS_FIN_LCAP : s_scalar[4];
        const bool over = s_scalar[4] > HS_FIN_LCAP;
        if (over) { s_scalar[3] = 1; }
        else {
            s_scalar[3] = 0;
            for (int i = 1; i < nl; ++i) {
                const int a1 = lc1[i], a2 = lc2[i]; const double ar = lr[i];
                int j = i;
                while (j > 0 && ar > lr[j - 1]) { lc1[j] = lc1[j - 1]; lc2[j] = lc2[j - 1]; lr[j] = lr[j - 1]; --j; }
                lc1[j] = a1; lc2[j] = a2; lr[j] = ar;
            }
            for (int x = 0; x < M; ++x) s_o2n[x] = 0;
            for (int i = 0; i < G; ++i) s_o2n[s_glist[i] + 2] = s_glist[i];
            s_o2n[1] = -1; s_o2n[0] = -2;
            for (int q = 0; q < nl; ++q) {
                if (!(lr[q] > 0.01)) continue;
                const int c1 = lc1[q], c2 = lc2[q];
                if (s_o2n[c1 + 2] == s_o2n[c2 + 2]) continue;
                bool bad = false;
                for (int i = 0; i < G; ++i) {
                    if (s_o2n[s_glist[i] + 2] != s_o2n[c1 + 2]) continue;
                    for (int k = 0; k < G; ++k)
                        if (s_o2n[s_glist[k] + 2] == s_o2n[c2 + 2] && s_incompat[s_gidx[i] * G + s_gidx[k]] > 1) bad = true;
                }
                if (!bad) { const int to = s_o2n[c1 + 2], from = s_o2n[c2 + 2]; for (int k = 0; k < G; ++k) if (s_o2n[s_glist[k] + 2] == from) s_o2n[s_glist[k] + 2] = to; }
            }
            for (int x = 0; x < M; ++x) s_new_index[x] = -1;
            int ni = 0;
            for (int i = 0; i < G; ++i) { const int v = s_o2n[s_glist[i] + 2]; if (s_new_index[v + 2] < 0) s_new_index[v + 2] = ni++; }
            for (int i = 0; i < G; ++i) s_o2n[s_glist[i] + 2] = s_new_index[s_o2n[s_glist[i] + 2] + 2];
        }
    }
    wave_lds_sync();
    if (s_scalar[3]) { bail(); return; }
    for (int j = lane; j < m; j += 64) lout[j] = s_o2n[lab[j] + 2];
    if (lane == 0) ok_out[c] = 1;
    HS_TQ(4)
}

}
```

hairsplitter_amd/csrc/hs_sr_backend.inc:

```
struct GraphRows {
    DBuf d_oo, d_n, d_wc, d_row0, d_ids, d_rw, d_bo, d_fe, d_rank, d_rank_off, d_pos_rank;
    bool by_pos = false;
    UploadPack pack;
    DBuf d_off, d_nbr, d_visit, d_visit_n, d_prog_info, d_prog_bytes, d_prog_steps, d_prog_adj;
    int64_t rows = 0, rows_dev = 0, total = 0;
    bool total_exact = true;
    int W = 0, max_m = 1;
    std::vector<int32_t> win_m;
    DBuf d_bits, d_amb, d_deg, d_scan, d_wmo, d_ltw, d_lti, d_ltj, d_wsim, d_wdiff, d_stage, d_src, d_len, d_dst, d_os, d_od, d_pb, d_pm, d_pi, d_pj;
    UploadPack pk_amb, pk_patch;
    HBuf h_amb, h_rows, h_deg, h_nbr;
    std::vector<int32_t> row_win;
    std::vector<int64_t> win_bits_off, win_mat_off;
    std::vector<int32_t> lt_w, lt_i, lt_j;
    int Wd = 0, Wmx = 0, rows_mx = 0;
    int row_waves = 0; int64_t n_late = 0;
    size_t amb_cap = 0;
    int64_t stage_cap = 0, stage_hint = 0;
    EventPair ev;
    bool timed = false, begun = false;
    const int32_t* d_sim = nullptr; const int32_t* d_diff = nullptr; int es = 1;
    std::vector<int64_t> ctg_out_off; std::vector<int32_t> ctg_n;
    float* k_ms = nullptr;
};
// ... 442 lines not shown
        d_diff.release(); d_diff.p = (char*)d_sim.p + sizeof(int32_t); d_diff.bytes = 0; d_diff.cap = 0; d_diff.view = true;
        if (front) {
            auto fill = [&](void* p, size_t bytes, unsigned v) {
                const long long n16 = (long long)((bytes + 15) / 16);
                if (n16) hipLaunchKernelGGL(hsdev::k_fill16, dim3((unsigned)std::min<long long>(256, n16 / 4096 + 1)), dim3(256), 0, stream, reinterpret_cast<uint4*>(p), n16, v);
            };
            fill(f.d_alt.p, pbytes, 0xffffffffu); fill(f.d_ref.p, pbytes, 0xffffffffu);
            fill(d_sim.p, (size_t)job.out_total * 8, (unsigned)hs::SrGraphTaps::kSentinel);
            HS_HIP(hipGetLastError());
        }
        if (int rc = kc.begin(HS_K_SNP_PLANES, stream)) return rc;
        if (int rc = snp_planes_launch(d_col_off.as<int64_t>(), d_col_idx.as<int32_t>(), d_col_code.as<uint8_t>(), f.d_sr.as<uint8_t>(), f.d_sa.as<uint8_t>(),
                                       f.d_sc.as<int32_t>(), f.d_cb.as<int64_t>(), f.d_po.as<int64_t>(), f.d_w.as<int32_t>(), f.d_pn.as<int32_t>(), f.d_bc.as<int32_t>(),
                                       f.d_bw.as<int32_t>(), f.blk_c.size(), (int32_t)job.snp_ref.size(), f.d_alt.as<uint64_t>(), f.d_ref.as<uint64_t>(), stream,
                                       by_pos ? f.d_rb.as<int64_t>() : nullptr, rng_lo, rng_hi)) return rc;
        if (int rc = kc.end(5 * (adopted ? adopted_entries : (int64_t)ch.col_idx.size()) + 2 * (int64_t)pbytes, stream)) return rc;
        if (int rc = f.ev.init()) return rc;
        HS_HIP(ev_rec(f.ev.a, stream));
        if (int rc = kc.begin(HS_K_SIMDIFF, stream)) return rc;
        if (int rc = simdiff_launch(f.d_alt.as<uint64_t>(), f.d_ref.as<uint64_t>(), f.d_po.as<int64_t>(), f.d_n.as<int32_t>(), f.d_w.as<int32_t>(),
                                    f.d_oo.as<int64_t>(), d_sim.as<int32_t>(), d_diff.as<int32_t>(), stream, f.t_c.as<int32_t>(), f.t_i.as<int32_t>(), f.t_j.as<int32_t>(), f.tc.size(), 2,
                                    by_pos ? f.d_rb.as<int64_t>() : nullptr, by_pos ? f.d_orig.as<int32_t>() : nullptr, rng_lo, rng_hi)) return rc;
        if (int rc = kc.end(2 * (int64_t)pbytes + 8 * job.out_total, stream)) return rc;
        HS_HIP(ev_rec(f.ev.b, stream));
        if (front) {
            front->alt.assign((size_t)job.plane_total, ~0ull); front->ref.assign((size_t)job.plane_total, ~0ull);
            front->matrix.assign((size_t)job.out_total * 2, 0);
            if (pbytes) { if (int rc = d2h_pinned(front->alt.data(), f.d_alt.p, pbytes, stream)) return rc; if (int rc = d2h_pinned(front->ref.data(), f.d_ref.p, pbytes, stream)) return rc; }
            if (job.out_total > 0) { if (int rc = d2h_pinned(front->matrix.data(), d_sim.p, (size_t)job.out_total * 8, stream)) return rc; }
        }
        return HS_OK;
    }

    hs::SrGraphTaps* front = nullptr;
    void tap_front(hs::SrGraphTaps* t) override { front = t; }
    struct Keep { int64_t stage_hint = 0; };
    Keep* keep = nullptr;
    PlaneRows plane_rows() const {
        PlaneRows pr;
        if (sd_flight) { pr.d_alt = sd_flight->d_alt.as<uint64_t>(); pr.d_ref = sd_flight->d_ref.as<uint64_t>(); pr.d_plane_off = sd_flight->d_po.as<int64_t>(); pr.d_words = sd_flight->d_w.as<int32_t>(); }
        return pr;
    }
    int build_graphs(const hs::SrWindowSet& ws, int64_t* rows_on_host, float* k_ms) override {
        if (int rc = build_graphs_begin(ws, k_ms)) return rc;
        return build_graphs_end(ws, rows_on_host);
    }
    bool two_phase_graphs() const override { return true; }
    int build_graphs_begin(const hs::SrWindowSet& ws, float* k_ms) override {
        const PlaneRows pr = plane_rows();
        if (keep) G.stage_hint = keep->stage_hint;
        return graph_rows_begin(d_sim.as<int32_t>(), d_diff.as<int32_t>(), sd_out_off, sd_n, ws, G, stream, k_ms, &kc, &pr, 2);
    }
    int build_graphs_end(const hs::SrWindowSet& ws, int64_t* rows_on_host) override {
        const int rc = graph_rows_end(ws, G, stream, rows_on_host, &kc);
        if (!rc) k5_waited = true;
        if (!rc && front) { front->rows_late = G.n_late; front->row_waves = G.row_waves; }
        if (keep) keep->stage_hint = G.stage_hint;
        return rc;
    }
    int fetch_graphs(std::vector<int64_t>& off, std::vector<int32_t>& nbr) override {
        if (G.rows > 0 && !G.total_exact) { int64_t t = 0; if (int rc = d2h_pinned(&t, G.d_off.as<int64_t>() + G.rows, 8, stream)) return rc; G.total = t; G.total_exact = true; }
        off.assign((size_t)G.rows + 1, 0); nbr.assign((size_t)G.total, 0);
        if (int rc = d2h_pinned(off.data(), G.d_off.p, off.size() * 8, stream)) return rc;
        if (G.total > 0) { if (int rc = d2h_pinned(nbr.data(), G.d_nbr.p, nbr.size() * 4, stream)) return rc; }
        return HS_OK;
    }

    static int lds_nodes(int max_m, int ints_per_node, int limit_bytes) {
        const int cap = ((std::max(max_m, 1) + 63) / 64) * 64;
        return std::min(cap, (limit_bytes / (ints_per_node * 4)) / 64 * 64);
    }

    std::vector<int64_t>* tap_run_off = nullptr; std::vector<int32_t>* tap_run_labels = nullptr; hs::SrChainRoutes* tap_routes = nullptr;
    void tap_chain(std::vector<int64_t>* run_off, std::vector<int32_t>* run_labels, hs::SrChainRoutes* routes) override { tap_run_off = run_off; tap_run_labels = run_labels; tap_routes = routes; }
    int cw_chain(const hs::CwChain& ch, std::vector<int32_t>& labels, std::vector<int32_t>& final_labels, std::vector<uint8_t>& final_ok,
                 float k_ms[3], hs::SrChainStats* stats) override {
        if (int rc = settle_simdiff()) return rc;
        const int Wc = (int)ch.win.size();
        const int64_t n_inst = (int64_t)ch.seed_col.size();
        const int64_t total_m = ch.chain_row0.back();
        if (n_inst > 0x7fffffff) { set_error("Chinese Whispers: too many runs in one call"); return HS_EINVAL; }
        std::vector<int32_t> inst_win((size_t)n_inst), list_big, list_lanes, unit_win, unit_inst0, unit_n;
        const int lanes_cap = 64;
        int max_m_small = 1;
        std::vector<int64_t> inst_slab((size_t)n_inst), chain_slab0((size_t)Wc), big_scr, tail_scr((size_t)Wc, 0);
        int64_t slab = 0, big_scr_total = 0, tail_scr_total = 0;
        int max_m_big = 1, max_m_chain = 1;
        bool all_lanes = true;
        for (int k = 0; k < Wc && all_lanes; ++k) all_lanes = G.win_m[(size_t)ch.win[(size_t)k]] <= lanes_cap;
        if (all_lanes) {
            for (int k = 0; k < Wc; ++k) {
                const int m = G.win_m[(size_t)ch.win[(size_t)k]];
                chain_slab0[(size_t)k] = slab;
                max_m_chain = std::max(max_m_chain, m);
                slab += (ch.win_seed_begin[(size_t)k + 1] - ch.win_seed_begin[(size_t)k]) * (int64_t)m;
            }
            list_lanes.resize((size_t)n_inst);
            hs::hs_parallel_for(Wc, std::min(8, host_threads()), [&](int k) {
                const int w = ch.win[(size_t)k];
                const int m = G.win_m[(size_t)w];
                int64_t sl = chain_slab0[(size_t)k];
                for (int64_t i = ch.win_seed_begin[(size_t)k]; i < ch.win_seed_begin[(size_t)k + 1]; ++i) { inst_win[(size_t)i] = w; inst_slab[(size_t)i] = sl; sl += m; list_lanes[(size_t)i] = (int32_t)i; }
            });
        } else
        for (int k = 0; k < Wc; ++k) {
            const int w = ch.win[(size_t)k];
            const int m = G.win_m[(size_t)w];
            chain_slab0[(size_t)k] = slab;
            max_m_chain = std::max(max_m_chain, m);
            for (int64_t i = ch.win_seed_begin[(size_t)k]; i < ch.win_seed_begin[(size_t)k + 1]; ++i) {
                inst_win[(size_t)i] = w; inst_slab[(size_t)i] = slab; slab += m;
                if (m > HS_CWR_CAP) { list_big.push_back((int32_t)i); max_m_big = std::max(max_m_big, m); }
                else if (m <= lanes_cap) list_lanes.push_back((int32_t)i);
            }
            if (m <= HS_CWR_CAP && m > lanes_cap) {
                max_m_small = std::max(max_m_small, m);
                for (int64_t i = ch.win_seed_begin[(size_t)k]; i < ch.win_seed_begin[(size_t)k + 1]; i += 8) {
                    unit_win.push_back(w); unit_inst0.push_back((int32_t)i);
                    unit_n.push_back((int32_t)std::min<int64_t>(8, ch.win_seed_begin[(size_t)k + 1] - i));
                }
            }
        }
        const int cap_big = lds_nodes(max_m_big, 2, 96 * 1024);
        for (int32_t i : list_big) {
            const int m = G.win_m[(size_t)inst_win[(size_t)i]];
            big_scr.push_back(big_scr_total);
            if (m > cap_big) big_scr_total += 2 * (int64_t)m;
        }
        const int cap_tail = lds_nodes(max_m_chain, 7, 56 * 1024);
        if (tap_routes) {
            hs::SrChainRoutes& rt = *tap_routes;
            rt = hs::SrChainRoutes();
            rt.all_lanes = all_lanes ? 1 : 0; rt.runs_lanes = (int64_t)list_lanes.size(); rt.units_rows = (int64_t)unit_win.size();
            for (int32_t n : unit_n) rt.runs_rows += n;
            rt.runs_wave = (int64_t)list_big.size();
            for (int32_t i : list_big) if (G.win_m[(size_t)inst_win[(size_t)i]] > cap_big) rt.runs_wave_scratch++;
            rt.cap_tail = cap_tail;
            for (int k = 0; k < Wc; ++k) { const int m = G.win_m[(size_t)ch.win[(size_t)k]]; if (m <= 64) rt.tail_narrow++; else if (m > cap_tail) rt.tail_scratch++; else rt.tail_lds++; }
        }
        std::vector<int32_t> tail_list((size_t)Wc);
        int n_tail_small = 0;
        {
            int wide = 0;
            for (int k = 0; k < Wc; ++k) if (G.win_m[(size_t)ch.win[(size_t)k]] <= 64) n_tail_small++;
            int at_small = 0;
            for (int k = 0; k < Wc; ++k) { if (G.win_m[(size_t)ch.win[(size_t)k]] <= 64) tail_list[(size_t)at_small++] = k; else tail_list[(size_t)(n_tail_small + wide++)] = k; }
        }
        for (int k = 0; k < Wc; ++k) {
            const int m = G.win_m[(size_t)ch.win[(size_t)k]];
            tail_scr[(size_t)k] = tail_scr_total;
            if (m > cap_tail) tail_scr_total += 7 * (int64_t)m + (m & 1);
        }
        DBuf d_ll, d_sets, d_names, d_slots, d_alive, d_ovf, d_ovf_n, d_iw, d_is, d_seed, d_uw, d_ui, d_un, d_lb, d_bs, d_cw, d_cr0, d_csb, d_cs0, d_ts, d_slab, d_gs, d_l3, d_final, d_ok, d_stat,
            d_cpos, d_sf, d_sl, d_plo, d_phi, d_tl;
        if (resident_cols != &ch && !adopted) {
            col_pack.add(ch.col_off, d_col_off); col_pack.add(ch.col_idx, d_col_idx); col_pack.add(ch.col_code, d_col_code);
            if (int rc = col_pack.commit(stream)) return rc;
            resident_cols = &ch;
        }
        const bool finish = ch.finish_on_device && !std::getenv("HS_FINISH_ON_HOST");
        UploadPack pk;
        pk.add(inst_win, d_iw); pk.add(inst_slab, d_is); pk.add(ch.seed_col, d_seed); pk.add(unit_win, d_uw); pk.add(unit_inst0, d_ui); pk.add(unit_n, d_un); pk.add(list_big, d_lb); pk.add(list_lanes, d_ll);
        pk.add(big_scr, d_bs); pk.add(ch.win, d_cw); pk.add(ch.chain_row0, d_cr0); pk.add(ch.win_seed_begin, d_csb); pk.add(chain_slab0, d_cs0);
        pk.add(tail_scr, d_ts); pk.add(tail_list, d_tl);
        if (finish) { pk.add(ch.col_pos, d_cpos); pk.add(ch.win_snp_first, d_sf); pk.add(ch.win_snp_last, d_sl); pk.add(ch.win_pos_lo, d_plo); pk.add(ch.win_pos_hi, d_phi); }
        if (int rc = pk.commit(stream)) return rc;
        if (int rc = d_slab.alloc(std::max<size_t>((size_t)slab, 1) * 4)) return rc;
        if (int rc = d_gs.alloc(std::max<size_t>((size_t)std::max(big_scr_total, tail_scr_total), 2) * 4)) return rc;
        if (int rc = d_l3.alloc(std::max<size_t>((size_t)total_m, 1) * 4)) return rc;
        if (int rc = d_final.alloc(std::max<size_t>((size_t)total_m, 1) * 4)) return rc;
        if (int rc = d_ok.alloc(std::max<size_t>((size_t)Wc, 1))) return rc;
        if (int rc = d_stat.alloc(416)) return rc;
        hipLaunchKernelGGL(hsdev::k_fill16, dim3(1), dim3(64), 0, stream, d_stat.as<uint4>(), 26ll, 0u);
        EventPair e1, e2;
        if (int rc = e1.init()) return rc;
        if (int rc = e2.init()) return rc;
        HS_HIP(ev_rec(e1.a, stream));
        if (!list_lanes.empty()) {
            const int n = (int)list_lanes.size();
            const size_t npad = ((size_t)n + 63) & ~(size_t)63;
            if (int rc = d_sets.alloc(npad * 128)) return rc;
            if (int rc = d_names.alloc(npad * 16)) return rc;
            if (int rc = d_slots.alloc(npad * 64)) return rc;
            if (int rc = d_alive.alloc(npad)) return rc;
            if (int rc = d_ovf.alloc((size_t)n * 4)) return rc;
            if (int rc = d_ovf_n.alloc(16)) return rc;
            hipLaunchKernelGGL(hsdev::k_fill16, dim3(1), dim3(64), 0, stream, d_ovf_n.as<uint4>(), 1ll, 0u);
            if (int rc = kc.begin(HS_K_CW_SEED_SETS, stream)) return rc;
            hipLaunchKernelGGL(hsdev::k_cw_seed_sets, dim3((unsigned)((n + 3) / 4)), dim3(256), 0, stream, G.d_row0.as<int64_t>(), G.d_ids.as<int32_t>(), d_ll.as<int32_t>(), n,
                               d_iw.as<int32_t>(), d_seed.as<int64_t>(), d_col_off.as<int64_t>(), d_col_idx.as<int32_t>(), d_col_code.as<uint8_t>(),
                               d_sets.as<unsigned long long>(), d_names.as<uint8_t>(), d_slots.as<uint8_t>(), d_alive.as<uint8_t>(), d_ovf.as<int32_t>(), d_ovf_n.as<int32_t>());
            HS_HIP(hipGetLastError());
            if (int rc = kc.end((int64_t)npad * 209 + 5 * (int64_t)n * 40, stream)) return rc;
            if (int rc = kc.begin(HS_K_CW_SEEDED, stream)) return rc;
            hipLaunchKernelGGL(hsdev::k_cw_seeded_lanes, dim3((unsigned)(npad / 64)), dim3(64), 0, stream, G.d_off.as<int64_t>(), G.d_row0.as<int64_t>(), G.d_visit_n.as<int32_t>(),
                               G.d_prog_info.as<uint32_t>(), G.d_prog_adj.as<unsigned long long>(), d_ll.as<int32_t>(), n, d_iw.as<int32_t>(), d_is.as<int64_t>(),
                               d_sets.as<unsigned long long>(), d_names.as<uint8_t>(), d_slots.as<uint8_t>(), d_alive.as<uint8_t>(), d_slab.as<int32_t>(), d_stat.as<unsigned long long>());
            HS_HIP(hipGetLastError());
            if (int rc = kc.end((int64_t)npad * 209, stream)) return rc;
            const bool timing = std::getenv("HS_TIMING") != nullptr;
            if (timing || tap_routes) {
                int32_t n_ovf = 0;
                if (int rc = d2h_pinned(&n_ovf, d_ovf_n.p, 4, stream)) return rc;
                if (tap_routes) tap_routes->runs_overflow = n_ovf;
                if (timing) {
                    std::fprintf(stderr, "[hs timing] sr: %d per-SNP runs one per lane, %d of them with more than 16 labels alive (-> one wavefront each); %zu runs in units of 8, %zu one wavefront each\n",
                                 n, n_ovf, unit_win.size() * 8, list_big.size());
                }
            }
            if (int rc = kc.begin(HS_K_CW_SEEDED_WIDE, stream)) return rc;
            hipLaunchKernelGGL(hsdev::k_cw_seeded_wave, dim3((unsigned)std::min(n, 1024)), dim3(64), (size_t)64 * 8, stream, G.d_off.as<int64_t>(), G.d_nbr.as<int32_t>(),
                               G.d_row0.as<int64_t>(), G.d_ids.as<int32_t>(), G.d_visit.as<int32_t>(), G.d_visit_n.as<int32_t>(), d_ovf.as<int32_t>(), 0, d_ovf_n.as<int32_t>(),
                               d_iw.as<int32_t>(), d_seed.as<int64_t>(), d_is.as<int64_t>(), d_col_off.as<int64_t>(), d_col_idx.as<int32_t>(),
                               d_col_code.as<uint8_t>(), 64, (int32_t*)nullptr, (const int64_t*)nullptr, d_slab.as<int32_t>(), d_stat.as<unsigned long long>());
            HS_HIP(hipGetLastError());
            if (int rc = kc.end(0, stream)) return rc;
        }
        if (!unit_win.empty() || !list_big.empty()) { if (int rc = kc.begin(HS_K_CW_SEEDED_WIDE, stream)) return rc; }
        if (!unit_win.empty()) {
            const int n = (int)unit_win.size();
            const int m_cap = std::max(16, (max_m_small + 15) & ~15);
            const int cnt_cap = std::max(m_cap, 256);
            const int prog_cap = std::max(2048, m_cap * 32);
            const size_t lds = (size_t)2 * m_cap * 4 + (size_t)8 * cnt_cap * 4 + (size_t)prog_cap + (size_t)8 * m_cap;
            if (lds > 48 * 1024)
                HS_HIP(hipFuncSetAttribute(reinterpret_cast<const void*>(hsdev::k_cw_seeded_rows), hipFuncAttributeMaxDynamicSharedMemorySize, (int)lds));
            hipLaunchKernelGGL(hsdev::k_cw_seeded_rows, dim3((unsigned)n), dim3(128), lds, stream, G.d_off.as<int64_t>(), G.d_nbr.as<int32_t>(),
                               G.d_row0.as<int64_t>(), G.d_ids.as<int32_t>(), G.d_visit.as<int32_t>(), G.d_visit_n.as<int32_t>(), G.d_prog_info.as<uint32_t>(),
                               G.d_prog_bytes.as<uint8_t>(), G.d_prog_steps.as<int32_t>(), d_uw.as<int32_t>(), d_ui.as<int32_t>(), d_un.as<int32_t>(), n, d_seed.as<int64_t>(), d_is.as<int64_t>(), d_col_off.as<int64_t>(), d_col_idx.as<int32_t>(),
                               d_col_code.as<uint8_t>(), m_cap, prog_cap, d_slab.as<int32_t>(), d_stat.as<unsigned long long>());
            HS_HIP(hipGetLastError());
        }
        if (!list_big.empty()) {
            const int n = (int)list_big.size();
            const size_t lds = (size_t)cap_big * 8;
            if (lds > 48 * 1024)
                HS_HIP(hipFuncSetAttribute(reinterpret_cast<const void*>(hsdev::k_cw_seeded_wave), hipFuncAttributeMaxDynamicSharedMemorySize, (int)lds));
            hipLaunchKernelGGL(hsdev::k_cw_seeded_wave, dim3((unsigned)n), dim3(64), lds, stream, G.d_off.as<int64_t>(), G.d_nbr.as<int32_t>(),
                               G.d_row0.as<int64_t>(), G.d_ids.as<int32_t>(), G.d_visit.as<int32_t>(), G.d_visit_n.as<int32_t>(), d_lb.as<int32_t>(), n, (const int32_t*)nullptr,
                               d_iw.as<int32_t>(), d_seed.as<int64_t>(), d_is.as<int64_t>(), d_col_off.as<int64_t>(), d_col_idx.as<int32_t>(),
                               d_col_code.as<uint8_t>(), cap_big, d_gs.as<int32_t>(), d_bs.as<int64_t>(), d_slab.as<int32_t>(), d_stat.as<unsigned long long>());
            HS_HIP(hipGetLastError());
        }
        if (!unit_win.empty() || !list_big.empty()) { if (int rc = kc.end(0, stream)) return rc; }
        HS_HIP(ev_rec(e1.b, stream));
        HS_HIP(ev_rec(e2.a, stream));
        if (int rc = kc.begin(HS_K_WINDOW_TAIL, stream)) return rc;
        if (Wc > 0) {
            const size_t lds = (size_t)cap_tail * 7 * 4 + HS_TAIL_MAP_EXTRA;
            if (lds > 32 * 1024)
                HS_HIP(hipFuncSetAttribute(reinterpret_cast<const void*>(hsdev::k_window_tail), hipFuncAttributeMaxDynamicSharedMemorySize, (int)lds));
            for (int part = 0; part < 2; ++part) {
                const int n_part = part == 0 ? n_tail_small : Wc - n_tail_small;
                if (n_part == 0) continue;
                const int cap = part == 0 ? std::min(cap_tail, 64) : cap_tail;
                hipLaunchKernelGGL(hsdev::k_window_tail, dim3((unsigned)n_part), dim3(64), (size_t)cap * 7 * 4 + HS_TAIL_MAP_EXTRA, stream, G.d_off.as<int64_t>(), G.d_nbr.as<int32_t>(), G.d_row0.as<int64_t>(),
                                   G.d_ids.as<int32_t>(), G.d_visit.as<int32_t>(), G.d_visit_n.as<int32_t>(), G.d_fe.as<uint8_t>(), G.d_prog_info.as<uint32_t>(),
                                   G.d_prog_adj.as<unsigned long long>(), d_cw.as<int32_t>(), d_cr0.as<int64_t>(),
                                   d_csb.as<int64_t>(), d_cs0.as<int64_t>(), d_slab.as<int32_t>(), d_tl.as<int32_t>() + (part == 0 ? 0 : n_tail_small), n_part, d_col_off.as<int64_t>(),
                                   d_col_idx.as<int32_t>(), d_col_code.as<uint8_t>(), d_cpos.as<int32_t>(), d_sf.as<int64_t>(), d_sl.as<int64_t>(), d_plo.as<int32_t>(), d_phi.as<int32_t>(),
                                   finish ? 1 : 0, cap, d_gs.as<int32_t>(), d_ts.as<int64_t>(), d_l3.as<int32_t>(), d_final.as<int32_t>(), d_ok.as<uint8_t>(),
                                   d_stat.as<unsigned long long>() + 2);
            }
            HS_HIP(hipGetLastError());
        }
        if (int rc = kc.end(4 * slab + 8 * total_m, stream)) return rc;
        HS_HIP(ev_rec(e2.b, stream));
        {
            HBuf h, h4;
            const size_t o_nnz = 416, o_final = 512, o_ok = o_final + (((size_t)total_m * 4 + 255) & ~(size_t)255);
            if (int rc = h4.alloc(o_ok + (size_t)Wc + 256)) return rc;
            Shipment sh;
            sh.add(h4.p, d_stat.p, 416);
            const int64_t* h_nnz = sh.add_word((char*)h4.p + o_nnz, G.d_off.as<int64_t>() + G.rows);
            bool need_chain_labels = !finish || tap_run_labels != nullptr;
            if (finish) {
                sh.add((char*)h4.p + o_final, d_final.p, (size_t)total_m * sizeof(int32_t));
                sh.add((char*)h4.p + o_ok, d_ok.p, (size_t)Wc);
            }
            if (int rc = kc.begin(HS_K_SHIP, stream)) return rc;
            if (int rc = sh.launch(stream, 64)) return rc;
            if (int rc = kc.end(0, stream)) return rc;
            if (int rc = stream_wait(stream)) return rc;
            if (finish) {
                final_labels.resize((size_t)total_m); final_ok.resize((size_t)Wc);
                std::memcpy(final_labels.data(), (const char*)h4.p + o_final, (size_t)total_m * sizeof(int32_t));
                std::memcpy(final_ok.data(), (const char*)h4.p + o_ok, (size_t)Wc);
                for (uint8_t ok : final_ok) if (!ok) { need_chain_labels = true; break; }
            }
            if (need_chain_labels) {
                labels.resize((size_t)total_m);
                if (int rc = h.alloc(std::max<size_t>((size_t)total_m, 1) * sizeof(int32_t))) return rc;
                if (int rc = copy_d2h(h.p, d_l3.p, (size_t)total_m * sizeof(int32_t), stream)) return rc;
                std::memcpy(labels.data(), h.p, (size_t)total_m * sizeof(int32_t));
            } else labels.clear();
            if (tap_run_labels && tap_run_off) {
                tap_run_labels->resize((size_t)slab);
                if (slab) { if (int rc = d2h_pinned(tap_run_labels->data(), d_slab.p, (size_t)slab * sizeof(int32_t), stream)) return rc; }
                tap_run_off->assign(inst_slab.begin(), inst_slab.end()); tap_run_off->push_back(slab);
            }
            if (!G.total_exact) { G.total = *h_nnz; G.total_exact = true; }
            if (int rc = graph_rows_settle(G, &kc)) return rc;
            const unsigned long long* st = (const unsigned long long*)h4.p;
            if (stats) { stats->n_instances = n_inst + 2 * (int64_t)Wc; stats->sweeps = (int64_t)(st[0] + st[2]); stats->bytes = (int64_t)(st[1] + st[3]); stats->graph_nnz = G.total; }
            if (std::getenv("HS_TIMING")) {
                std::string h;
                for (int k = 0; k < 16; ++k) h += " " + std::to_string((unsigned long long)st[4 + k]);
                std::fprintf(stderr, "[hs timing] sr: per-SNP Chinese-Whispers runs by number of sweeps (0..15+):%s\n", h.c_str());
#ifdef HS_TAIL_DIAG
                std::fprintf(stderr, "[hs timing] sr: k_window_tail cycles: merged ids %llu, two runs + small clusters %llu, renumbering %llu, merge_close_clusters %llu, merge_wrongly_split_haplotypes: slots + map %llu, SNPs %llu, link counts %llu, links + output %llu; SNPs fast %llu slow %llu, keys %llu, windows with map %llu, clusters %llu\n",
                             (unsigned long long)st[20], (unsigned long long)st[21], (unsigned long long)st[22], (unsigned long long)st[23], (unsigned long long)st[25], (unsigned long long)st[26],
                             (unsigned long long)st[27], (unsigned long long)st[24], (unsigned long long)st[28], (unsigned long long)st[29], (unsigned long long)st[30], (unsigned long long)st[31], (unsigned long long)st[32]);
#endif
#ifdef HS_CW_DIAG
                h.clear(); for (int k = 0; k < 16; ++k) h += " " + std::to_string((unsigned long long)st[20 + k]);
                std::fprintf(stderr, "[hs timing] sr: runs by labels alive after seeding (0..15+):%s\n", h.c_str());
                h.clear(); for (int k = 0; k < 16; ++k) h += " " + std::to_string((unsigned long long)st[36 + k]);
                std::fprintf(stderr, "[hs timing] sr: runs by m/16:%s\n", h.c_str());
#endif
            }
            KernelClock::add_bytes(HS_K_CW_SEEDED, (int64_t)st[1]);
            KernelClock::add_bytes(HS_K_WINDOW_TAIL, (int64_t)st[3]);
            kc.flush();
        }
        float m = 0;
        if (int rc = e1.ms(&m)) return rc; k_ms[0] += m;
        if (int rc = e2.ms(&m)) return rc; k_ms[1] += m;
        return HS_OK;
    }
    int cw(hs::CwWave& wv, float* k_ms) override {
        const int n_inst = (int)wv.inst_win.size();
        if (n_inst == 0) return HS_OK;
        int max_m = 1;
        for (int w : wv.inst_win) max_m = std::max(max_m, G.win_m[(size_t)w]);
        const int cap = lds_nodes(max_m, 2, 96 * 1024);
        std::vector<int64_t> scr((size_t)n_inst, 0);
        int64_t scr_total = 0;
        for (int k = 0; k < n_inst; ++k) { const int m = G.win_m[(size_t)wv.inst_win[(size_t)k]]; scr[(size_t)k] = scr_total; if (m > cap) scr_total += 2 * (int64_t)m; }
        DBuf d_iw, d_lo, d_lab, d_scr, d_gs;
        UploadPack pk;
        pk.add(wv.inst_win, d_iw); pk.add(wv.inst_label_off, d_lo); pk.add(wv.labels, d_lab); pk.add(scr, d_scr);
        if (int rc = pk.commit(stream)) return rc;
        if (int rc = d_gs.alloc(std::max<size_t>((size_t)scr_total, 2) * 4)) return rc;
        EventPair ev; if (int rc = ev.init()) return rc;
        HS_HIP(ev_rec(ev.a, stream));
        if (int rc = kc.begin(HS_K_CW_LOCAL, stream)) return rc;
        const size_t lds = (size_t)cap * 8;
        if (lds > 48 * 1024)
            HS_HIP(hipFuncSetAttribute(reinterpret_cast<const void*>(hsdev::k_cw_local), hipFuncAttributeMaxDynamicSharedMemorySize, (int)lds));
        hipLaunchKernelGGL(hsdev::k_cw_local, dim3((unsigned)n_inst), dim3(64), lds, stream, G.d_off.as<int64_t>(), G.d_nbr.as<int32_t>(), G.d_row0.as<int64_t>(),
                           G.d_visit.as<int32_t>(), G.d_visit_n.as<int32_t>(), G.d_fe.as<uint8_t>(), d_iw.as<int32_t>(), d_lo.as<int64_t>(), n_inst, cap,
                           d_gs.as<int32_t>(), d_scr.as<int64_t>(), d_lab.as<int32_t>());
        HS_HIP(hipGetLastError());
        if (int rc = kc.end(8 * (int64_t)wv.labels.size(), stream)) return rc;
        HS_HIP(ev_rec(ev.b, stream));
        if (int rc = d2h_pinned(wv.labels.data(), d_lab.p, wv.labels.size() * sizeof(int32_t), stream)) return rc;
        float m = 0; if (int rc = ev.ms(&m)) return rc;
        if (k_ms) *k_ms += m;
        return HS_OK;
    }
};

}
```

include/hairsplitter_hip.h:

```cpp
#ifndef HAIRSPLITTER_HIP_H
#define HAIRSPLITTER_HIP_H

#include <stddef.h>
#include <stdint.h>

#ifdef __cplusplus
extern "C" {
#endif

#define HS_OK 0
#define HS_ENODEVICE (-1)
#define HS_EINVAL (-2)
#define HS_EHIP (-3)
#define HS_EIO (-4)
#define HS_EFORMAT (-5)

const char* hs_version(void);
const char* hs_last_error(void);
int hs_device_count(void);
int hs_warmup(void);
int hs_set_device(int device);
int hs_device_synchronize(void);
int hs_malloc(void** d_ptr, size_t bytes);
int hs_free(void* d_ptr);
// ... 181 lines not shown
typedef struct hs_cv_result {
    int32_t n_contigs;
    float* mean_distance;
    float* depth;
    int64_t* snp_off;
    int32_t* snp_pos;
    uint8_t* snp_ref;
    uint8_t* snp_alt;
    int32_t* snp_n_ref;
    int32_t* snp_n_alt;
    int64_t* col_off;
    int32_t* col_idx;
    uint8_t* col_code;
    float error_rate;
    int32_t n_contigs_with_error_rate;
    double t_device_ms;
    double t_host_ms;
    float t_kernel_ms[4];
    float t_kernel_k4_ms;
    int64_t n_columns_extracted;
    int64_t n_columns_downloaded;
    int64_t n_columns_downloaded_late;
    int32_t entries_borrowed;
} hs_cv_result;

int hs_cv_run(hs_cv_batch* b, float automatic_snp_threshold, int32_t n_threads, hs_cv_result** out);

typedef struct hs_cand_bits {
    int32_t wlo; uint16_t n_words, n_slots; int32_t idx_min, idx_max, reach, n_entries; int64_t word_off;
} hs_cand_bits;
typedef struct hs_cv_taps {
    int32_t n_contigs;
    int64_t n_cols, n_entries;
    int64_t* col_gpos;
    hs_colrec* col_rec;
    int64_t* col_off;
    int32_t* col_idx;
    uint8_t* col_code;
    int64_t n_cand;
    hs_colrec* cand_rec;
    int32_t* cand_col;
    hs_cand_bits* cand_bits;
    uint64_t* cand_words;
    int64_t n_cand_words;
    int32_t* contig_n_cand;
    float* contig_mean_distance;
} hs_cv_taps;
int hs_cv_column_pass_taps(hs_cv_batch* b, int32_t c0, int32_t c1, float automatic_snp_threshold, hs_cv_taps** out);
void hs_cv_taps_destroy(hs_cv_taps* t);

typedef struct hs_cv_pileup_taps {
    int32_t n_rec;
    int32_t pile_lead;
    int64_t pile_alloc_bytes;
    int64_t n_chunks;
    uint8_t* pile;
    int64_t* pile_addr;
    int32_t* rec_stats;
    int64_t* rec_chunk_off;
    int32_t* chunk_table;
} hs_cv_pileup_taps;
int hs_cv_pileup_tap(hs_cv_batch* b, int32_t c0, int32_t c1, int32_t fill, hs_cv_pileup_taps** out);
void hs_cv_pileup_tap_destroy(hs_cv_pileup_taps* t);

int hs_devices(int32_t* out, int32_t cap);
int hs_cv_run_host(const uint8_t* h_contig_seq, const int64_t* h_contig_off, int32_t n_contigs,
                   const uint8_t* h_read_seq, const int64_t* h_read_off, int32_t n_reads,
                   const int32_t* h_rec_read, const int32_t* h_rec_pos, const uint8_t* h_rec_strand,
                   const int64_t* h_rec_cig_off, const uint32_t* h_cigar, const int32_t* h_contig_rec_off,
                   float automatic_snp_threshold, int32_t n_threads, hs_cv_result** out);

typedef struct hs_cv_selection {
    int64_t n_selected;
    float t_kernel_ms[4];
    double t_device_ms, t_host_ms;
    void* impl;
} hs_cv_selection;
int hs_cv_select(hs_cv_batch* b, hs_cv_selection** out);
int hs_cv_run_range(hs_cv_batch* b, const hs_cv_selection* sel, int32_t c0, int32_t c1, float automatic_snp_threshold,
                    int32_t n_threads, hs_cv_result** out);
void hs_cv_selection_destroy(hs_cv_selection* sel);
void hs_cv_result_destroy(hs_cv_result* r);

typedef struct hs_sr_contig {
    int64_t length;
    int32_t n_reads;
    const int32_t* read_start;
    const int32_t* read_end;
    int32_t n_snps;
    const int32_t* snp_pos;
    const uint8_t* snp_ref;
    const uint8_t* snp_alt;
    const int64_t* col_off;
    const int32_t* col_idx;
    const uint8_t* col_code;
    int32_t ploidy;
} hs_sr_contig;

typedef struct hs_sr_result {
    int32_t n_contigs;
    int64_t* win_off;
    int32_t* win_start;
    int32_t* win_end;
    int64_t* label_off;
    int32_t* labels;
    double t_device_ms;
    double t_host_ms;
    int64_t n_cw_instances;
    float t_kernel_ms[4];
    float t_kernel_graph_ms;
    int64_t n_graph_rows_host;
    int64_t n_windows_finished_on_host;
    int64_t n_cw_sweeps;
    int64_t cw_bytes;
    int64_t graph_nnz;
    int64_t n_graph_rows;
    int64_t simdiff_bytes;
} hs_sr_result;

int hs_sr_run(const hs_sr_contig* contigs, int32_t n_contigs, int32_t window_size, float error_rate,
              int32_t low_memory, uint32_t seed, int32_t n_threads, hs_sr_result** out);

typedef struct hs_sr_taps {
    int32_t n_windows;
    int32_t* win_contig; int32_t* win_start;
    int64_t* win_row0;
    int32_t* mask_ids;
    int64_t* run_begin;
    int32_t* run_snp;
    int64_t* run_off;
    int32_t* run_labels;
    int32_t* third;
    int32_t g_n_windows;
    int32_t* g_win_contig; int32_t* g_win_kind;
    int64_t* g_win_row0;
    int32_t* g_mask_ids;
    int64_t* g_nbr_off; int32_t* g_nbr;
    int32_t g_n_contigs;
    int32_t* g_plane_n; int32_t* g_words;
    int64_t* g_plane_off;
    uint64_t* g_alt; uint64_t* g_ref;
    int32_t* g_n_reads; int64_t* g_out_off;
    int64_t* g_read_base; int32_t* g_pos_orig;
    int64_t g_n_pos_orig, g_n_plane_words, g_n_pairs;
    int32_t* g_matrix;
    int64_t g_rows_on_host, g_rows_late;
    int32_t g_row_waves;
    int32_t all_lanes;
    int32_t cap_tail;
    int64_t runs_lanes, runs_overflow;
    int64_t runs_rows, units_rows;
    int64_t runs_wave, runs_wave_scratch;
    int64_t tail_narrow, tail_lds, tail_scratch;
} hs_sr_taps;
#define HS_SR_TAPS_CHAIN 0
#define HS_SR_TAPS_GRAPHS 1
#define HS_SR_TAP_SENTINEL INT32_MIN
int hs_sr_run_taps(const hs_sr_contig* contigs, int32_t n_contigs, int32_t window_size, float error_rate, int32_t low_memory, uint32_t seed,
                   int32_t n_threads, int32_t mode, hs_sr_result** out, hs_sr_taps** taps);
void hs_sr_taps_destroy(hs_sr_taps* t);
void hs_sr_result_destroy(hs_sr_result* r);
int hs_sr_run_cv_range(const hs_cv_batch* b, int32_t c0, int32_t c1, const hs_cv_result* cv, float error_rate,
                       float rarest_strain_abundance, int32_t low_memory, int32_t amplicon, uint32_t seed, int32_t n_threads,
                       int32_t window_size, hs_sr_result** out);
int hs_sr_run_cv(const hs_cv_batch* b, const hs_cv_result* cv, float error_rate, float rarest_strain_abundance,
                 int32_t low_memory, int32_t amplicon, uint32_t seed, int32_t n_threads, int32_t window_size,
                 hs_sr_result** out);

typedef struct hs_allele_cell { uint16_t n, best, second, n_ref, n_alt; uint8_t best_code, call; } hs_allele_cell;
typedef struct hs_allele_table {
    int64_t n_windows, n_snps, n_groups, n_cells;
    int32_t *win_contig, *win_start, *win_end;
    int64_t* win_group_off;
    int32_t* group_ids;
    int64_t* win_snp_off;
    int32_t *snp_contig, *snp_pos;
    uint8_t *snp_ref, *snp_alt;
    int32_t* snp_n_calls;
    int64_t* snp_cell_off;
    hs_allele_cell* cells;
    double t_kernel_ms;
    int64_t n_entries;
    int64_t n_wide_columns;
} hs_allele_table;
void hs_allele_table_destroy(hs_allele_table* t);
int hs_alleles_text(const hs_allele_table* t, const char* const* names, int32_t n_names, char** out);
int32_t hs_alleles_lds_capacity(void);
typedef struct hs_allele_layout { int64_t snp_win, grp_n, win_snp_first, win_snp_last, cell_off, grp_off, n_calls, grp_ids, grp_pack, internal, total_bytes; } hs_allele_layout;
int hs_group_alleles_layout(int32_t n_snps, int32_t n_windows, int64_t n_labels, hs_allele_layout* out);
int hs_group_alleles(const int64_t* d_col_off, const int32_t* d_col_idx, const uint8_t* d_col_code,
                     const uint8_t* d_snp_ref, const uint8_t* d_snp_alt, const int32_t* d_snp_pos, const int32_t* d_snp_contig, int32_t n_snps,
                     const int64_t* d_win_off , const int32_t* d_win_start, const int32_t* d_win_end, int32_t n_contigs, int32_t n_windows,
                     const int64_t* d_label_off , const int32_t* d_labels, int64_t n_labels,
                     void* d_work, hs_allele_cell* d_cells, int64_t cells_cap, void* stream);
int hs_haplotype_alleles(const hs_sr_contig* contigs, int32_t n_contigs, const hs_sr_result* sr_result, hs_allele_table** table);

#define HS_RECRUIT_ABSENT 1
#define HS_RECRUIT_UNCLUSTERED 2
#define HS_RECRUIT_LABELLED 4
typedef struct hs_recruit_params { int32_t which, min_informative, min_margin, mismatch_num, mismatch_den; } hs_recruit_params;
hs_recruit_params hs_recruit_params_default(void);
typedef struct hs_recruit_row {
    int32_t read, label, best_group, second_group;
    uint32_t m_best, x_best, m_second, x_second, n_entries;
    int32_t assigned;
} hs_recruit_row;
typedef struct hs_recruit_table {
    int64_t n_windows, n_rows, n_assigned;
    int32_t *win_contig, *win_start, *win_end;
    int64_t* win_index;
    int64_t* win_row_off;
    hs_recruit_row* rows;
    hs_recruit_params params;
    int64_t n_call_windows;
    int64_t n_counter_words;
    int64_t n_entries;
    double t_kernel_ms;
} hs_recruit_table;
void hs_recruit_table_destroy(hs_recruit_table* t);
int hs_recruit_reads(const hs_sr_contig* contigs, int32_t n_contigs, const hs_sr_result* sr_result, const hs_recruit_params* params,
                     hs_allele_table** alleles, hs_recruit_table** out);
typedef struct hs_recruit_layout { hs_allele_layout alleles; int64_t flag, row_idx, ctr_off, win_row_off, status, internal, total_bytes; } hs_recruit_layout;
int hs_group_recruit_layout(int32_t n_snps, int32_t n_windows, int64_t n_labels, hs_recruit_layout* out);
int hs_group_recruit(const int64_t* d_col_off, const int32_t* d_col_idx, const uint8_t* d_col_code,
                     const uint8_t* d_snp_ref, const uint8_t* d_snp_alt, const int32_t* d_snp_pos, const int32_t* d_snp_contig, int32_t n_snps,
                     const int64_t* d_win_off, const int32_t* d_win_start, const int32_t* d_win_end, int32_t n_contigs, int32_t n_windows,
                     const int64_t* d_label_off, const int32_t* d_labels, int64_t n_labels, const hs_recruit_params* params,
                     void* d_work, hs_allele_cell* d_cells, int64_t cells_cap, uint32_t* d_counters, int64_t counters_cap,
                     hs_recruit_row* d_rows, int64_t rows_cap, void* stream);
int hs_recruit_apply(const hs_recruit_table* table, const int64_t* label_off, const int32_t* labels_in, int32_t* labels_out, int64_t n_labels);
int hs_recruit_text(const hs_recruit_table* t, const char* const* names, int32_t n_names, char** out);

typedef struct hs_pipeline hs_pipeline;
typedef struct hs_pipeline_stats {
    int64_t n_snps, n_cw_instances, n_graph_rows_host;
    double t_device_ms, t_host_ms;
    float t_kernel_cv_ms[4];
    float t_kernel_k4_ms;
    float t_kernel_sr_ms[4];
    float t_kernel_graph_ms;
    int64_t n_columns_extracted, n_columns_downloaded, n_columns_downloaded_late;
    int64_t n_cw_sweeps, cw_bytes, graph_nnz, n_graph_rows, simdiff_bytes;
} hs_pipeline_stats;
int hs_pipeline_create(hs_cv_batch* b, int32_t n_groups, hs_pipeline** out);
int hs_pipeline_select(hs_pipeline* p, float* mean_distance , hs_pipeline_stats* stats);
int hs_pipeline_run(hs_pipeline* p, float automatic_snp_threshold, float error_rate, float rarest_strain_abundance, int32_t low_memory,
                    int32_t amplicon, uint32_t seed, int32_t n_threads, int32_t window_size, hs_sr_result** out,
                    hs_pipeline_stats* stats);
int hs_pipeline_run_fused(hs_pipeline* p, float automatic_snp_threshold, float rarest_strain_abundance, int32_t low_memory, int32_t amplicon,
                          uint32_t seed, int32_t n_threads, int32_t window_size, float* mean_distance, float* error_rate_out, hs_sr_result** out,
                          hs_pipeline_stats* st);
int hs_pipeline_thread_devices(hs_pipeline* p, int32_t* out, int32_t cap);
#define HS_PIPELINE_KEEP_COLUMNS 1
#define HS_PIPELINE_SPARSE_LABELS 2
#define HS_PIPELINE_ALLELES 4
const hs_allele_table* hs_pipeline_alleles(const hs_pipeline* p);
#define HS_PIPELINE_RECRUIT 8
const hs_recruit_table* hs_pipeline_recruits(const hs_pipeline* p);
int hs_pipeline_set_recruit_params(hs_pipeline* p, const hs_recruit_params* params);
int hs_pipeline_set_option(hs_pipeline* p, int32_t option, int64_t value);
int hs_pipeline_groups(const hs_pipeline* p);
int hs_pipeline_group_range(const hs_pipeline* p, int32_t g, int32_t* c0, int32_t* c1);
int hs_pipeline_sparse_labels(const hs_pipeline* p, const int64_t** win_row_off, const int32_t** ids, const int32_t** labels, int64_t* n_windows, int64_t* n_rows);
const hs_cv_result* hs_pipeline_group_cv(const hs_pipeline* p, int32_t g);
void hs_pipeline_destroy(hs_pipeline* p);

int32_t hs_sr_window_size(const hs_sr_contig* contigs, int32_t n_contigs, int32_t amplicon);

int hs_call_variants_main(int argc, char** argv);
void hs_call_variants_epilogue(void);
int hs_separate_reads_main(int argc, char** argv);
void hs_main_process_exits(int yes);

int hs_gaf_from_files(const char* gfa, const char* reads, const char* sam, const char* gro, int32_t amplicon, const char* out_gaf,
                      int32_t n_threads);
int hs_gaf_from_labels(const char* gfa, const char* reads, const char* sam, int32_t amplicon, int32_t n_contigs,
                       const int64_t* win_off, const int32_t* win_start, const int32_t* win_end, const int64_t* label_off,
                       const int32_t* labels, const uint8_t* contig_has_snps, const char* out_gaf, int32_t n_threads);
int hs_gro_to_gaf_main(int argc, char** argv);

#define HS_POLISH_START_BEYOND_SEQ 2
typedef struct hs_polish_result {
    int64_t n_bundles, n_pieces, n_dropped;
    int32_t *bundle_contig, *bundle_interval , *bundle_start, *bundle_end, *bundle_group,
        *bundle_left_to_polish, *bundle_right_to_polish, *bundle_overhang_left, *bundle_overhang_right;
    int64_t* backbone_off;
    uint8_t* backbone;
    int64_t* piece_off;
    int32_t *piece_rec , *piece_read_start, *piece_read_end ,
        *piece_sam_pos , *piece_flags;
    int64_t* base_off;
    uint8_t* bases;
    int64_t* cig_off;
    uint32_t* cigar;
    int32_t* dropped;
    double t_scan_ms, t_cut_ms, t_gather_ms, t_cigar_ms;
    int64_t n_tasks, n_rounds, cut_ops_read;
} hs_polish_result;
int hs_polish_inputs(hs_cv_batch* b, int32_t c0, int32_t c1, const int64_t* win_off, const int32_t* win_start, const int32_t* win_end,
                     const int64_t* label_off, const int32_t* labels, const uint8_t* contig_has_snps, int32_t polish_everything,
                     hs_polish_result** out);
int hs_polish_inputs_from_files(const char* gfa, const char* reads, const char* sam, const char* gro, int32_t polish_everything,
                                const char* out_path, int32_t n_threads);
void hs_polish_result_destroy(hs_polish_result* r);
int hs_polish_inputs_main(int argc, char** argv);

// ... 101 lines not shown
```

Measured before the change: 131.9 billion.

## Reuse seed-run clustering records to score tail SNPs instead of rewalking columns

The seed-sets kernel now also stores, per seeded run, the allele code of each cluster and a flag saying whether every read in the column was covered. In the window-tail kernel, SNP columns that have a usable record compute per-group majority alleles directly from the stored cluster bitsets, so they skip re-reading col_idx/col_code and re-running the per-SNP walk. Those SNPs feed the pair-incompatibility counts in column order alongside the walked ones. This adds extra buffers, an instance-to-seed index upload, per-block seed column scanning and more register/LDS use in the tail kernel. The path is on by default and can be disabled with an environment variable.

```diff
diff --git a/hairsplitter_amd/api.py b/hairsplitter_amd/api.py
--- a/hairsplitter_amd/api.py
+++ b/hairsplitter_amd/api.py
@@ -692,11 +692,12 @@
                 ("g_matrix", C.POINTER(C.c_int32)), ("g_rows_on_host", C.c_int64), ("g_rows_late", C.c_int64), ("g_row_waves", C.c_int32),
                 ("all_lanes", C.c_int32), ("cap_tail", C.c_int32), ("runs_lanes", C.c_int64), ("runs_overflow", C.c_int64), ("runs_rows", C.c_int64),
                 ("units_rows", C.c_int64), ("runs_wave", C.c_int64), ("runs_wave_scratch", C.c_int64), ("tail_narrow", C.c_int64), ("tail_lds", C.c_int64),
-                ("tail_scratch", C.c_int64)]
+                ("tail_scratch", C.c_int64), ("tail_snps_seeded", C.c_int64), ("tail_snps_walked", C.c_int64)]
 
 
 SR_ROUTE_COUNTERS = ("all_lanes", "runs_lanes", "runs_overflow", "runs_rows", "units_rows", "runs_wave", "runs_wave_scratch", "tail_narrow", "tail_lds",
                      "tail_scratch", "cap_tail")
+SR_TAIL_COUNTERS = ("tail_snps_seeded", "tail_snps_walked")
 
 
 SR_TAP_SENTINEL = -2 ** 31
@@ -767,7 +768,7 @@
     out = {"win_contig": a(t.win_contig, Wc, np.int32), "win_start": a(t.win_start, Wc, np.int32), "win_row0": row0, "mask_ids": a(t.mask_ids, int(row0[-1]), np.int32),
            "run_begin": rb, "run_snp": a(t.run_snp, n_runs, np.int32), "run_off": ro, "run_labels": a(t.run_labels, int(ro[-1]), np.int32),
            "third": a(t.third, int(row0[-1]), np.int32)}
-    for k in SR_ROUTE_COUNTERS:
+    for k in SR_ROUTE_COUNTERS + SR_TAIL_COUNTERS:
         out[k] = int(getattr(t, k))
     return out
 
diff --git a/hairsplitter_amd/csrc/hs_capi_multi.inc b/hairsplitter_amd/csrc/hs_capi_multi.inc
--- a/hairsplitter_amd/csrc/hs_capi_multi.inc
+++ b/hairsplitter_amd/csrc/hs_capi_multi.inc
@@ -79,7 +79,7 @@
         const hs::SrChainRoutes& rt = tp.routes;
         t->all_lanes = rt.all_lanes; t->cap_tail = rt.cap_tail; t->runs_lanes = rt.runs_lanes; t->runs_overflow = rt.runs_overflow; t->runs_rows = rt.runs_rows;
         t->units_rows = rt.units_rows; t->runs_wave = rt.runs_wave; t->runs_wave_scratch = rt.runs_wave_scratch; t->tail_narrow = rt.tail_narrow;
-        t->tail_lds = rt.tail_lds; t->tail_scratch = rt.tail_scratch;
+        t->tail_lds = rt.tail_lds; t->tail_scratch = rt.tail_scratch; t->tail_snps_seeded = rt.tail_snps_seeded; t->tail_snps_walked = rt.tail_snps_walked;
     }
     if (tp.graphs) {
         const hs::SrGraphTaps& f = tp.front;
diff --git a/hairsplitter_amd/csrc/hs_driver.h b/hairsplitter_amd/csrc/hs_driver.h
--- a/hairsplitter_amd/csrc/hs_driver.h
+++ b/hairsplitter_amd/csrc/hs_driver.h
@@ -167,6 +167,8 @@
     int64_t tail_lds = 0;
     int64_t tail_scratch = 0;
     int32_t cap_tail = 0;
+    int64_t tail_snps_seeded = 0;
+    int64_t tail_snps_walked = 0;
 };
 struct SrDeviceOps {
     virtual ~SrDeviceOps() {}
diff --git a/hairsplitter_amd/csrc/hs_kernels_cw.hip b/hairsplitter_amd/csrc/hs_kernels_cw.hip
--- a/hairsplitter_amd/csrc/hs_kernels_cw.hip
+++ b/hairsplitter_amd/csrc/hs_kernels_cw.hip
@@ -415,14 +415,18 @@
     const int32_t* __restrict__ col_idx, const uint8_t* __restrict__ col_code,
     unsigned long long* __restrict__ seed_sets , uint8_t* __restrict__ seed_names ,
     uint8_t* __restrict__ seed_slots , uint8_t* __restrict__ seed_n ,
+    uint8_t* __restrict__ seed_codes ,
+    uint8_t* __restrict__ seed_use ,
     int32_t* __restrict__ ovf_list, int32_t* __restrict__ ovf_n) {
     __shared__ int32_t s_ids[4][64];
     __shared__ int32_t s_lab[4][64];
     __shared__ int32_t s_first[4][256];
+    __shared__ uint8_t s_code[4][64];
     const int lane = (int)threadIdx.x & 63, wv = (int)threadIdx.x >> 6;
     const int q = (int)blockIdx.x * 4 + wv;
     if (q >= n_list) return;
     int32_t* ids = s_ids[wv]; int32_t* lab = s_lab[wv]; int32_t* first = s_first[wv];
+    uint8_t* code_of = s_code[wv];
     const int inst = inst_list[q];
     const int w = inst_win[inst];
     const int64_t seed = inst_seed_col[inst];
@@ -434,11 +438,13 @@
     const int code0 = e0 < c1 ? (int)col_code[e0] : 0;
     ids[lane] = lane < m ? mask_ids[r0 + lane] : 0x7fffffff;
     lab[lane] = lane;
+    code_of[lane] = 0xff;
     for (int c = lane; c < 256; c += 64) first[c] = 0x7fffffff;
     wave_lds_sync();
     const int j0 = R0 >= 0 ? local_index(ids, m, R0) : -1;
-    if (j0 >= 0) atomicMin(&first[code0], j0);
-    for (int64_t e = e0 + 64; e < c1; e += 64) { const int j = local_index(ids, m, col_idx[e]); if (j >= 0) atomicMin(&first[col_code[e]], j); }
+    if (j0 >= 0) { atomicMin(&first[code0], j0); code_of[j0] = (uint8_t)code0; }
+    int n_deep = 0;
+    for (int64_t e = e0 + 64; e < c1; e += 64) { const int j = local_index(ids, m, col_idx[e]); if (j >= 0) { atomicMin(&first[col_code[e]], j); code_of[j] = col_code[e]; n_deep++; } }
     wave_lds_sync();
     if (j0 >= 0) lab[j0] = first[code0];
     for (int64_t e = e0 + 64; e < c1; e += 64) { const int j = local_index(ids, m, col_idx[e]); if (j >= 0) lab[j] = first[col_code[e]]; }
@@ -450,7 +456,7 @@
     const int slot = __popcll(leaders & ((1ull << L) - 1ull));
     seed_slots[(int64_t)q * 64 + lane] = (uint8_t)(node ? slot : 0);
     if (alive > HS_CWL_SLOTS) {
-        if (lane == 0) { seed_n[q] = 255; ovf_list[atomicAdd(ovf_n, 1)] = inst; }
+        if (lane == 0) { seed_n[q] = 255; seed_use[q] = 0; ovf_list[atomicAdd(ovf_n, 1)] = inst; }
         return;
     }
     unsigned long long mine = 0ull;
@@ -461,6 +467,11 @@
     wave_lds_sync();
     if (lane < HS_CWL_SLOTS) seed_names[(int64_t)q * HS_CWL_SLOTS + lane] = (uint8_t)(lane < alive ? ids[lane] : 0);
     if (lane == 0) seed_n[q] = (uint8_t)alive;
+    if (lane < HS_CWL_SLOTS) seed_codes[(int64_t)q * HS_CWL_SLOTS + lane] = lane < alive ? code_of[ids[lane]] : (uint8_t)0xff;
+    int n_in = __popcll(__ballot(j0 >= 0));
+    if (c1 - c0 > 64) n_in += wave_sum_i32(n_deep);
+    const int n_coded = __popcll(__ballot(node && code_of[lane] != 0xff));
+    if (lane == 0) seed_use[q] = n_coded == n_in ? 1 : 0;
 }
 
 template <int NS>
@@ -699,7 +710,12 @@
     const int32_t* __restrict__ col_pos, const int64_t* __restrict__ win_snp_first, const int64_t* __restrict__ win_snp_last,
     const int32_t* __restrict__ win_pos_lo, const int32_t* __restrict__ win_pos_hi, int finish_on_device,
     int lds_cap, int32_t* __restrict__ gscratch, const int64_t* __restrict__ gscratch_off,
-    int32_t* __restrict__ labels3_out, int32_t* __restrict__ final_out, uint8_t* __restrict__ ok_out, unsigned long long* __restrict__ stat) {
+    int32_t* __restrict__ labels3_out, int32_t* __restrict__ final_out, uint8_t* __restrict__ ok_out, unsigned long long* __restrict__ stat,
+    const unsigned long long* __restrict__ seed_sets ,
+    const uint8_t* __restrict__ seed_codes, const uint8_t* __restrict__ seed_n, const uint8_t* __restrict__ seed_use,
+    const int64_t* __restrict__ seed_col ,
+    const int32_t* __restrict__ inst_q ,
+    unsigned long long* __restrict__ route_stat ) {
     extern __shared__ int32_t tail_dyn[];
     __shared__ int s_count[HS_FIN_KCAP], s_initial[HS_FIN_KCAP], s_tested[HS_FIN_KCAP];
     __shared__ int s_index_of[HS_FIN_KCAP], s_slot_of[HS_FIN_KCAP];
@@ -1051,7 +1067,7 @@
     const bool pair_owner = lane < G * G && s_glist[pa] > s_glist[pb];
     int pair_inc = 0, pair_last = -10;
 #ifdef HS_TAIL_DIAG
-    unsigned long long dq_fast = 0, dq_slow = 0, dq_keys = 0;
+    unsigned long long dq_fast = 0, dq_slow = 0, dq_keys = 0, dq_seeded = 0;
 #endif
     auto pairs_update = [&](int p, int major) {
         const bool counts_l = lane < G && major != 0 && major != ' ';
@@ -1131,6 +1147,46 @@
         }
         pairs_update(p, major);
     };
+    const bool seeded_on = masks && seed_sets != nullptr;
+    auto snp_records = [&](int rq) -> bool {
+        unsigned long long Sg = 0ull;
+        {
+            const int gl = lane < G ? s_glist[lane] : 0;
+            const unsigned lo = (unsigned)__shfl((int)(unsigned)fin_S, gl, 64), hi = (unsigned)__shfl((int)(unsigned)(fin_S >> 32), gl, 64);
+            if (lane < G) Sg = ((unsigned long long)hi << 32) | lo;
+        }
+        const bool mine = rq >= 0;
+        const int64_t rb = (int64_t)(mine ? rq : 0) * HS_CWL_SLOTS;
+        const int n_mine = mine ? (int)seed_n[rq] : 0;
+        const uint4 cw = reinterpret_cast<const uint4*>(seed_codes)[mine ? rq : 0];
+        const int n_max = wave_max_i32(n_mine);
+        unsigned maj_lo = 0u, maj_hi = 0u, first_max = 0u;
+        bool several = false;
+#pragma nounroll
+        for (int i = 0; i < G; ++i) {
+            const unsigned long long Si = readlane_u64(Sg, i);
+            int t1v = 0, t2v = 0, c1 = 0, nbv = 0;
+#pragma nounroll
+            for (int s = 0; s < n_max; ++s) {
+                const unsigned w = s < 4 ? cw.x : s < 8 ? cw.y : s < 12 ? cw.z : cw.w;
+                const int cd = (int)((w >> (8 * (s & 3))) & 255u);
+                const unsigned long long set = (s < n_mine && cd != 0xff) ? seed_sets[rb + s] : 0ull;
+                const int v = __popcll(set & Si);
+                nbv += v;
+                if (v > t1v) { t2v = t1v; t1v = v; c1 = cd; } else if (v > t2v) t2v = v;
+            }
+            unsigned major = 0u;
+            if (t1v > 0) { major = (unsigned)c1; if (t2v * 2 > t1v || nbv * 0.5 > t1v) major = (unsigned)' '; }
+            if (i < 4) maj_lo |= major << (8 * i); else maj_hi |= major << (8 * (i - 4));
+            if (major != 0u && major != (unsigned)' ') { if (first_max == 0u) first_max = major; else several = several || major != first_max; }
+        }
+        s_sets[lane] = ((unsigned long long)maj_hi << 32) | maj_lo;
+        wave_lds_sync();
+        return several;
+    };
+    const int64_t csb = chain_seed_begin[c];
+    int jb = 0;
+    int n_seeded = 0, n_walked = 0;
     for (int64_t sb = win_snp_first[c]; sb < win_snp_last[c]; sb += 64) {
         const int64_t s_l = sb + lane;
         const bool s_valid = s_l < win_snp_last[c];
@@ -1139,6 +1195,41 @@
         const int n_l = s_valid ? (int)(col_off[s_l + 1] - e0_l) : 0;
         unsigned long long todo = __ballot(s_valid && p_l >= pos_lo && p_l < pos_hi);
         auto rl_e0 = [&](int l) { return ((int64_t)(unsigned)__builtin_amdgcn_readlane((int)(e0_l >> 32), l) << 32) | (unsigned)__builtin_amdgcn_readlane((int)(e0_l & 0xffffffffll), l); };
+        int run_q = -1;
+        if (seeded_on) {
+            unsigned long long sm = 0ull;
+            for (;;) {
+                const int64_t cs = jb + lane < K ? seed_col[csb + jb + lane] : 0x7fffffffffffffffll;
+                const int behind = __popcll(__ballot(cs < sb));
+                if (behind) { jb += behind; continue; }
+                sm = wave_or_u64(cs < sb + 64 ? 1ull << (int)((cs - sb) & 63) : 0ull);
+                break;
+            }
+            if ((sm >> lane) & 1ull) {
+                const int64_t inst = csb + jb + __popcll(sm & ((1ull << lane) - 1ull));
+                const int rq = inst_q ? inst_q[inst] : (int)inst;
+                if (rq >= 0 && seed_use[rq]) run_q = rq;
+            }
+            jb += __popcll(sm);
+        }
+        const unsigned long long from_record = __ballot(run_q >= 0);
+        n_seeded += __popcll(todo & from_record); n_walked += __popcll(todo & ~from_record);
+        unsigned long long todo_rec = 0ull;
+        if (from_record) { const bool several = snp_records(run_q); todo_rec = todo & from_record & __ballot(several); }
+#ifdef HS_TAIL_DIAG
+        dq_seeded += (unsigned long long)__popcll(todo & from_record);
+#endif
+        auto records_before = [&](int a_end) {
+            while (todo_rec) {
+                const int a = __builtin_ctzll(todo_rec);
+                if (a >= a_end) break;
+                todo_rec &= todo_rec - 1ull;
+                const unsigned long long wd = s_sets[a];
+                const int ma = (int)((wd >> (8 * pa)) & 255ull), mb = (int)((wd >> (8 * pb)) & 255ull), p = __builtin_amdgcn_readlane(p_l, a);
+                if (pair_owner && ma != ' ' && mb != ' ' && ma != mb && p - pair_last > 10) { pair_inc += 1; pair_last = p; }
+            }
+        };
+        todo &= ~from_record;
         while (todo) {
             int aq[HS_TAIL_BATCH], idx_b[HS_TAIL_BATCH], code_b[HS_TAIL_BATCH];
             bool any_deep = false;
@@ -1159,6 +1250,7 @@
 #pragma unroll
                 for (int q = 0; q < HS_TAIL_BATCH; ++q) {
                     if (aq[q] < 0) break;
+                    records_before(aq[q]);
                     snp_fast(__builtin_amdgcn_readlane(p_l, aq[q]), __builtin_amdgcn_readlane(n_l, aq[q]), idx_b[q], code_b[q]);
                 }
             } else {
@@ -1168,14 +1260,18 @@
                     bt &= bt - 1ull;
                     const int p = __builtin_amdgcn_readlane(p_l, a), n = __builtin_amdgcn_readlane(n_l, a);
                     const int64_t e0 = rl_e0(a);
+                    records_before(a);
                     if (n <= 64) { int idx = -1, code = 0; if (lane < n) { idx = col_idx[e0 + lane]; code = col_code[e0 + lane]; } snp_fast(p, n, idx, code); }
                     else snp_deep(p, e0, n);
                 }
             }
         }
-    }
+        records_before(64);
+        wave_lds_sync();
+    }
+    if (route_stat && lane == 0) { atomicAdd(&route_stat[0], (unsigned long long)n_seeded); atomicAdd(&route_stat[1], (unsigned long long)n_walked); }
 #ifdef HS_TAIL_DIAG
-    if (lane == 0 && stat) { atomicAdd(&stat[18 + 8], dq_fast); atomicAdd(&stat[18 + 9], dq_slow); atomicAdd(&stat[18 + 10], dq_keys); atomicAdd(&stat[18 + 11], use_map ? 1ull : 0ull); atomicAdd(&stat[18 + 12], (unsigned long long)G); }
+    if (lane == 0 && stat) { atomicAdd(&stat[18 + 8], dq_fast); atomicAdd(&stat[18 + 9], dq_slow); atomicAdd(&stat[18 + 10], dq_keys); atomicAdd(&stat[18 + 11], use_map ? 1ull : 0ull); atomicAdd(&stat[18 + 12], (unsigned long long)G); atomicAdd(&stat[18 + 13], dq_seeded); }
 #endif
     if (pair_owner) { const int i1 = s_gidx[pa], i2 = s_gidx[pb]; s_incompat[i1 * G + i2] = pair_inc; s_incompat[i2 * G + i1] = pair_inc; }
     wave_lds_sync();
diff --git a/hairsplitter_amd/csrc/hs_sr_backend.inc b/hairsplitter_amd/csrc/hs_sr_backend.inc
--- a/hairsplitter_amd/csrc/hs_sr_backend.inc
+++ b/hairsplitter_amd/csrc/hs_sr_backend.inc
@@ -618,17 +618,25 @@
             if (m > cap_tail) tail_scr_total += 7 * (int64_t)m + (m & 1);
         }
         DBuf d_ll, d_sets, d_names, d_slots, d_alive, d_ovf, d_ovf_n, d_iw, d_is, d_seed, d_uw, d_ui, d_un, d_lb, d_bs, d_cw, d_cr0, d_csb, d_cs0, d_ts, d_slab, d_gs, d_l3, d_final, d_ok, d_stat,
-            d_cpos, d_sf, d_sl, d_plo, d_phi, d_tl;
+            d_cpos, d_sf, d_sl, d_plo, d_phi, d_tl, d_iq;
         if (resident_cols != &ch && !adopted) {
             col_pack.add(ch.col_off, d_col_off); col_pack.add(ch.col_idx, d_col_idx); col_pack.add(ch.col_code, d_col_code);
             if (int rc = col_pack.commit(stream)) return rc;
             resident_cols = &ch;
         }
         const bool finish = ch.finish_on_device && !std::getenv("HS_FINISH_ON_HOST");
+        const char* tail_seeded_env = std::getenv("HS_TAIL_SEEDED");
+        const bool tail_seeded = !(tail_seeded_env && tail_seeded_env[0] == '0') && finish && !list_lanes.empty();
+        std::vector<int32_t> inst_q;
+        if (tail_seeded && !all_lanes) {
+            inst_q.assign((size_t)n_inst, -1);
+            for (size_t q = 0; q < list_lanes.size(); ++q) inst_q[(size_t)list_lanes[q]] = (int32_t)q;
+        }
         UploadPack pk;
         pk.add(inst_win, d_iw); pk.add(inst_slab, d_is); pk.add(ch.seed_col, d_seed); pk.add(unit_win, d_uw); pk.add(unit_inst0, d_ui); pk.add(unit_n, d_un); pk.add(list_big, d_lb); pk.add(list_lanes, d_ll);
         pk.add(big_scr, d_bs); pk.add(ch.win, d_cw); pk.add(ch.chain_row0, d_cr0); pk.add(ch.win_seed_begin, d_csb); pk.add(chain_slab0, d_cs0);
         pk.add(tail_scr, d_ts); pk.add(tail_list, d_tl);
+        if (!inst_q.empty()) pk.add(inst_q, d_iq);
         if (finish) { pk.add(ch.col_pos, d_cpos); pk.add(ch.win_snp_first, d_sf); pk.add(ch.win_snp_last, d_sl); pk.add(ch.win_pos_lo, d_plo); pk.add(ch.win_pos_hi, d_phi); }
         if (int rc = pk.commit(stream)) return rc;
         if (int rc = d_slab.alloc(std::max<size_t>((size_t)slab, 1) * 4)) return rc;
@@ -636,17 +644,18 @@
         if (int rc = d_l3.alloc(std::max<size_t>((size_t)total_m, 1) * 4)) return rc;
         if (int rc = d_final.alloc(std::max<size_t>((size_t)total_m, 1) * 4)) return rc;
         if (int rc = d_ok.alloc(std::max<size_t>((size_t)Wc, 1))) return rc;
-        if (int rc = d_stat.alloc(416)) return rc;
-        hipLaunchKernelGGL(hsdev::k_fill16, dim3(1), dim3(64), 0, stream, d_stat.as<uint4>(), 26ll, 0u);
+        if (int rc = d_stat.alloc(432)) return rc;
+        hipLaunchKernelGGL(hsdev::k_fill16, dim3(1), dim3(64), 0, stream, d_stat.as<uint4>(), 27ll, 0u);
         EventPair e1, e2;
         if (int rc = e1.init()) return rc;
         if (int rc = e2.init()) return rc;
         HS_HIP(ev_rec(e1.a, stream));
+        const size_t seed_npad = (list_lanes.size() + 63) & ~(size_t)63;
         if (!list_lanes.empty()) {
             const int n = (int)list_lanes.size();
-            const size_t npad = ((size_t)n + 63) & ~(size_t)63;
+            const size_t npad = seed_npad;
             if (int rc = d_sets.alloc(npad * 128)) return rc;
-            if (int rc = d_names.alloc(npad * 16)) return rc;
+            if (int rc = d_names.alloc(npad * 33)) return rc;
             if (int rc = d_slots.alloc(npad * 64)) return rc;
             if (int rc = d_alive.alloc(npad)) return rc;
             if (int rc = d_ovf.alloc((size_t)n * 4)) return rc;
@@ -655,9 +664,10 @@
             if (int rc = kc.begin(HS_K_CW_SEED_SETS, stream)) return rc;
             hipLaunchKernelGGL(hsdev::k_cw_seed_sets, dim3((unsigned)((n + 3) / 4)), dim3(256), 0, stream, G.d_row0.as<int64_t>(), G.d_ids.as<int32_t>(), d_ll.as<int32_t>(), n,
                                d_iw.as<int32_t>(), d_seed.as<int64_t>(), d_col_off.as<int64_t>(), d_col_idx.as<int32_t>(), d_col_code.as<uint8_t>(),
-                               d_sets.as<unsigned long long>(), d_names.as<uint8_t>(), d_slots.as<uint8_t>(), d_alive.as<uint8_t>(), d_ovf.as<int32_t>(), d_ovf_n.as<int32_t>());
-            HS_HIP(hipGetLastError());
-            if (int rc = kc.end((int64_t)npad * 209 + 5 * (int64_t)n * 40, stream)) return rc;
+                               d_sets.as<unsigned long long>(), d_names.as<uint8_t>(), d_slots.as<uint8_t>(), d_alive.as<uint8_t>(), d_names.as<uint8_t>() + npad * 16,
+                               d_names.as<uint8_t>() + npad * 32, d_ovf.as<int32_t>(), d_ovf_n.as<int32_t>());
+            HS_HIP(hipGetLastError());
+            if (int rc = kc.end((int64_t)npad * 226 + 5 * (int64_t)n * 40, stream)) return rc;
             if (int rc = kc.begin(HS_K_CW_SEEDED, stream)) return rc;
             hipLaunchKernelGGL(hsdev::k_cw_seeded_lanes, dim3((unsigned)(npad / 64)), dim3(64), 0, stream, G.d_off.as<int64_t>(), G.d_row0.as<int64_t>(), G.d_visit_n.as<int32_t>(),
                                G.d_prog_info.as<uint32_t>(), G.d_prog_adj.as<unsigned long long>(), d_ll.as<int32_t>(), n, d_iw.as<int32_t>(), d_is.as<int64_t>(),
@@ -726,7 +736,10 @@
                                    d_csb.as<int64_t>(), d_cs0.as<int64_t>(), d_slab.as<int32_t>(), d_tl.as<int32_t>() + (part == 0 ? 0 : n_tail_small), n_part, d_col_off.as<int64_t>(),
                                    d_col_idx.as<int32_t>(), d_col_code.as<uint8_t>(), d_cpos.as<int32_t>(), d_sf.as<int64_t>(), d_sl.as<int64_t>(), d_plo.as<int32_t>(), d_phi.as<int32_t>(),
                                    finish ? 1 : 0, cap, d_gs.as<int32_t>(), d_ts.as<int64_t>(), d_l3.as<int32_t>(), d_final.as<int32_t>(), d_ok.as<uint8_t>(),
-                                   d_stat.as<unsigned long long>() + 2);
+                                   d_stat.as<unsigned long long>() + 2,
+                                   tail_seeded ? d_sets.as<unsigned long long>() : (const unsigned long long*)nullptr, tail_seeded ? d_names.as<uint8_t>() + seed_npad * 16 : (const uint8_t*)nullptr,
+                                   tail_seeded ? d_alive.as<uint8_t>() : (const uint8_t*)nullptr, tail_seeded ? d_names.as<uint8_t>() + seed_npad * 32 : (const uint8_t*)nullptr, d_seed.as<int64_t>(),
+                                   inst_q.empty() ? (const int32_t*)nullptr : d_iq.as<int32_t>(), tap_routes ? d_stat.as<unsigned long long>() + 52 : (unsigned long long*)nullptr);
             }
             HS_HIP(hipGetLastError());
         }
@@ -734,10 +747,10 @@
         HS_HIP(ev_rec(e2.b, stream));
         {
             HBuf h, h4;
-            const size_t o_nnz = 416, o_final = 512, o_ok = o_final + (((size_t)total_m * 4 + 255) & ~(size_t)255);
+            const size_t o_nnz = 432, o_final = 512, o_ok = o_final + (((size_t)total_m * 4 + 255) & ~(size_t)255);
             if (int rc = h4.alloc(o_ok + (size_t)Wc + 256)) return rc;
             Shipment sh;
-            sh.add(h4.p, d_stat.p, 416);
+            sh.add(h4.p, d_stat.p, 432);
             const int64_t* h_nnz = sh.add_word((char*)h4.p + o_nnz, G.d_off.as<int64_t>() + G.rows);
             bool need_chain_labels = !finish || tap_run_labels != nullptr;
             if (finish) {
@@ -768,15 +781,16 @@
             if (!G.total_exact) { G.total = *h_nnz; G.total_exact = true; }
             if (int rc = graph_rows_settle(G, &kc)) return rc;
             const unsigned long long* st = (const unsigned long long*)h4.p;
+            if (tap_routes) { tap_routes->tail_snps_seeded = (int64_t)st[52]; tap_routes->tail_snps_walked = (int64_t)st[53]; }
             if (stats) { stats->n_instances = n_inst + 2 * (int64_t)Wc; stats->sweeps = (int64_t)(st[0] + st[2]); stats->bytes = (int64_t)(st[1] + st[3]); stats->graph_nnz = G.total; }
             if (std::getenv("HS_TIMING")) {
                 std::string h;
                 for (int k = 0; k < 16; ++k) h += " " + std::to_string((unsigned long long)st[4 + k]);
                 std::fprintf(stderr, "[hs timing] sr: per-SNP Chinese-Whispers runs by number of sweeps (0..15+):%s\n", h.c_str());
 #ifdef HS_TAIL_DIAG
-                std::fprintf(stderr, "[hs timing] sr: k_window_tail cycles: merged ids %llu, two runs + small clusters %llu, renumbering %llu, merge_close_clusters %llu, merge_wrongly_split_haplotypes: slots + map %llu, SNPs %llu, link counts %llu, links + output %llu; SNPs fast %llu slow %llu, keys %llu, windows with map %llu, clusters %llu\n",
+                std::fprintf(stderr, "[hs timing] sr: k_window_tail cycles: merged ids %llu, two runs + small clusters %llu, renumbering %llu, merge_close_clusters %llu, merge_wrongly_split_haplotypes: slots + map %llu, SNPs %llu, link counts %llu, links + output %llu; SNPs fast %llu slow %llu from the runs' record %llu, keys %llu, windows with map %llu, clusters %llu\n",
                              (unsigned long long)st[20], (unsigned long long)st[21], (unsigned long long)st[22], (unsigned long long)st[23], (unsigned long long)st[25], (unsigned long long)st[26],
-                             (unsigned long long)st[27], (unsigned long long)st[24], (unsigned long long)st[28], (unsigned long long)st[29], (unsigned long long)st[30], (unsigned long long)st[31], (unsigned long long)st[32]);
+                             (unsigned long long)st[27], (unsigned long long)st[24], (unsigned long long)st[28], (unsigned long long)st[29], (unsigned long long)st[33], (unsigned long long)st[30], (unsigned long long)st[31], (unsigned long long)st[32]);
 #endif
 #ifdef HS_CW_DIAG
                 h.clear(); for (int k = 0; k < 16; ++k) h += " " + std::to_string((unsigned long long)st[20 + k]);
diff --git a/include/hairsplitter_hip.h b/include/hairsplitter_hip.h
--- a/include/hairsplitter_hip.h
+++ b/include/hairsplitter_hip.h
@@ -357,6 +357,7 @@
     int64_t runs_rows, units_rows;
     int64_t runs_wave, runs_wave_scratch;
     int64_t tail_narrow, tail_lds, tail_scratch;
+    int64_t tail_snps_seeded, tail_snps_walked;
 } hs_sr_taps;
 #define HS_SR_TAPS_CHAIN 0
 #define HS_SR_TAPS_GRAPHS 1
```

Result: slower. 117.5 billion (-10.9%).
